# scychon/openmm_drudeNose

Hardware: AMD Instinct MI355X
Metric: integrator steps/sec at 1M Drude pairs (higher is better)
Workload: dtype f64; 1 GPU; SWM4-NDP water box, 1000000 molecules = 5000000 particle slots, 1000000 Drude pairs, 1 temperature group (+ molecular-COM and Drude thermostats), TGNH mode, mixed precision, numNHChains=1, hard wall 0.02 nm, harness force call-out inside the timed region (harness_force: lattice); harness_force=lattice, precision=mixed, variant=resident, hipgraph=False, parallelism=particle-sharded x1 (whole molecules), one KE all-reduce per step, slots_per_gpu=5000000

## Files before the change

### include/drude_tgnh.h

```cpp
#ifndef DRUDE_TGNH_H_
#define DRUDE_TGNH_H_

#include <stdint.h>

#ifdef __cplusplus
extern "C" {
#endif

#define TGNH_ABI_VERSION 1

typedef int tgnh_status;
enum {
    TGNH_OK = 0,
    TGNH_ERR_ARG = -1,
    TGNH_ERR_GROUP_MISMATCH = -2,
    TGNH_ERR_HARDWALL = -3,
    TGNH_ERR_UNSUPPORTED = -4,
    TGNH_ERR_HIP = -5,
    TGNH_ERR_STATE = -6
};

enum { TGNH_MODE_DUALNH = 0,
       TGNH_MODE_TGNH = 1 };

enum { TGNH_PREC_SINGLE = 0,
       TGNH_PREC_MIXED = 1,
       TGNH_PREC_DOUBLE = 2 };

enum { TGNH_FLAG_DEFER_SCALE = 2 };
enum { TGNH_FLAG_WAVE_TILES = 8 };
enum { TGNH_FLAG_RESIDENT_STEP = 4 };

enum { TGNH_FLAG_TRUST_STATE_CHANGED = 16 };

enum { TGNH_FLAG_GATHER = 32 };

typedef struct tgnh_desc {
    uint32_t struct_size;
    int32_t mode;
    int32_t precision;
    int32_t flags;
    int32_t device;
    int32_t num_particles;
    int32_t padded_num_particles;
    int32_t num_pairs;
    int32_t num_groups;
    int32_t num_residues;
    int32_t num_constraints;
    int32_t has_cm_motion_remover;
    const double* mass;
    const int32_t* pair_drude;
    const int32_t* pair_parent;
    const int32_t* group;
    const int32_t* resid;
    const int32_t* constraint_i;
    const int32_t* constraint_j;
    double kB;
    double temperature, coupling_time;
    double drude_temperature, drude_coupling_time;
    double step_size;
    int32_t drude_steps_per_real_step;
    int32_t num_nh_chains;
    int32_t use_drude_nh_chains;
    int32_t use_com_temp_group;
    double max_drude_distance;
} tgnh_desc;

typedef struct tgnh_context* tgnh_handle;


typedef int (*tgnh_allreduce_fn)(void* buf, int count, void* stream, void* user);

const char* tgnh_last_error(void);
int tgnh_abi_version(void);

tgnh_status tgnh_create(const tgnh_desc* desc, tgnh_handle* out);
tgnh_status tgnh_destroy(tgnh_handle h);

tgnh_status tgnh_bind_buffers(tgnh_handle h, void* posq, void* posq_correction, void* velm,
                              const void* force, void* pos_delta);

tgnh_status tgnh_set_step_size(tgnh_handle h, double dt);
tgnh_status tgnh_set_drude_steps_per_real_step(tgnh_handle h, int n);
tgnh_status tgnh_set_max_drude_distance(tgnh_handle h, double d);

tgnh_status tgnh_get_local_dof_terms(tgnh_handle h, double* terms, int* count);
tgnh_status tgnh_set_global_dof_terms(tgnh_handle h, const double* terms, int count);
tgnh_status tgnh_set_allreduce(tgnh_handle h, tgnh_allreduce_fn fn, void* user);

#define TGNH_RCCL_ID_BYTES 128
tgnh_status tgnh_rccl_unique_id(void* id_out);
tgnh_status tgnh_rccl_init(tgnh_handle h, int world, int rank, const void* id);
tgnh_status tgnh_set_rccl_comm(tgnh_handle h, void* nccl_comm);
tgnh_status tgnh_rccl_shutdown(tgnh_handle h);
tgnh_status tgnh_set_resident_share(tgnh_handle h, int share);
tgnh_status tgnh_get_resident_work_groups(tgnh_handle h, int* per_compute_unit);
tgnh_status tgnh_get_step_path(tgnh_handle h, int* gather, const char** reason);
tgnh_status tgnh_get_resident_kernel(tgnh_handle h, int* which);

#define TGNH_XCHG_HANDLE_BYTES 64
tgnh_status tgnh_exchange_create(tgnh_handle h, int world, int rank, void* ipc_handle_out, void** mailbox_out);
tgnh_status tgnh_exchange_attach(tgnh_handle h, const void* ipc_handles);
tgnh_status tgnh_exchange_attach_pointers(tgnh_handle h, void* const* mailboxes);
tgnh_status tgnh_exchange_detach(tgnh_handle h);
tgnh_status tgnh_exchange_wait_stats(tgnh_handle h, void* stream, double* mean_us, double* max_us, int64_t* exchanges);

tgnh_status tgnh_step_begin(tgnh_handle h, void* stream);
tgnh_status tgnh_step_end(tgnh_handle h, void* stream);
tgnh_status tgnh_step_begin_kick(tgnh_handle h, void* stream);
tgnh_status tgnh_step_begin_move(tgnh_handle h, void* stream);
tgnh_status tgnh_step_end_kick(tgnh_handle h, void* stream);
tgnh_status tgnh_step_end_thermo(tgnh_handle h, void* stream);
tgnh_status tgnh_flush(tgnh_handle h, void* stream);
tgnh_status tgnh_note_replayed_steps(tgnh_handle h, int nsteps);
tgnh_status tgnh_get_pending_state(tgnh_handle h, uint32_t* bits);
tgnh_status tgnh_set_time(tgnh_handle h, double time, int64_t step_count);
tgnh_status tgnh_state_changed(tgnh_handle h);

tgnh_status tgnh_get_kinetic_energy(tgnh_handle h, int ke_sum_valid, void* stream, double* out);
tgnh_status tgnh_get_num_thermostats(tgnh_handle h, int* count);
tgnh_status tgnh_get_last_kinetic_energies(tgnh_handle h, void* stream, double* ke);
tgnh_status tgnh_get_last_scale_factors(tgnh_handle h, void* stream, double* scale);
tgnh_status tgnh_get_status_flags(tgnh_handle h, void* stream, uint32_t* flags);
tgnh_status tgnh_get_time(tgnh_handle h, double* time, int64_t* step_count);
tgnh_status tgnh_get_dof(tgnh_handle h, double* dof, double* nkt);

tgnh_status tgnh_get_thermostat_len(tgnh_handle h, int which, int* len);
tgnh_status tgnh_get_thermostat_state(tgnh_handle h, int which, void* stream, double* out);
tgnh_status tgnh_set_thermostat_state(tgnh_handle h, int which, void* stream, const double* in);

tgnh_status tgnh_get_topology_len(tgnh_handle h, int which, int* len);
tgnh_status tgnh_get_topology(tgnh_handle h, int which, int32_t* out);
tgnh_status tgnh_get_launch_bounds(tgnh_handle h, int32_t out[8]);

tgnh_status tgnh_compute_kinetic_energies(tgnh_handle h, void* stream);
tgnh_status tgnh_half_kick(tgnh_handle h, void* stream);

tgnh_status tgnh_harness_force(tgnh_handle h, const void* x0, double k_drude, double k_tether,
                               void* force_out, void* stream);
tgnh_status tgnh_harness_pack_sites(tgnh_handle h, const void* x0);
tgnh_status tgnh_harness_lattice_hint(tgnh_handle h, int mol_slots, int side, double spacing, const double* geom, int first_molecule);
tgnh_status tgnh_harness_sites_kind(tgnh_handle h, int* kind);
tgnh_status tgnh_run_steps(tgnh_handle h, int nsteps, void* stream);
tgnh_status tgnh_run_harness(tgnh_handle h, const void* x0, double k_drude, double k_tether,
                             int nsteps, void* stream);

tgnh_status tgnh_harness_set_clusters(tgnh_handle h, int n, const int32_t* atoms, const double* dist);
tgnh_status tgnh_harness_shake_positions(tgnh_handle h, double tol, void* stream);
tgnh_status tgnh_harness_shake_velocities(tgnh_handle h, double tol, void* stream);
tgnh_status tgnh_harness_set_virtual_sites(tgnh_handle h, int n, const int32_t* atoms, const double* weights);
tgnh_status tgnh_harness_virtual_sites(tgnh_handle h, void* stream);
tgnh_status tgnh_run_harness_constrained(tgnh_handle h, const void* x0, double k_drude, double k_tether,
                                         double tol, int nsteps, void* stream);

tgnh_status tgnh_harness_water_force(tgnh_handle h, double box, double cutoff, void* force_out, void* stream);
tgnh_status tgnh_harness_remove_cm_motion(tgnh_handle h, void* stream);

tgnh_status tgnh_timing_enable(tgnh_handle h, int on);
tgnh_status tgnh_timing_read(tgnh_handle h, int kernel, double* total_ms, int64_t* launches);
tgnh_status tgnh_algorithmic_bytes(tgnh_handle h, int kernel, double* bytes);

#ifdef __cplusplus
}
#endif
#endif
```

### openmm_drudenose_amd/_lib.py

```python
import ctypes as C
import os

HERE = os.path.dirname(os.path.abspath(__file__))
LIB_PATH = os.environ.get("TGNH_LIB") or os.path.join(HERE, "libdrudetgnh_hip.so")

TGNH_OK = 0
ERR_ARG, ERR_GROUP_MISMATCH, ERR_HARDWALL, ERR_UNSUPPORTED, ERR_HIP, ERR_STATE = -1, -2, -3, -4, -5, -6
MODE_DUALNH, MODE_TGNH = 0, 1
PREC_SINGLE, PREC_MIXED, PREC_DOUBLE = 0, 1, 2
FLAG_DEFER_SCALE, FLAG_RESIDENT_STEP, FLAG_WAVE_TILES, FLAG_TRUST_STATE_CHANGED, FLAG_GATHER = 2, 4, 8, 16, 32
KID_SKD, KID_KICK_KE, KID_SCALE, KID_KE, KID_CHAIN, KID_FORCE, KID_OTHER, KID_STEP = range(8)
KERNEL_NAMES = {KID_SKD: "scale+kick+drift", KID_KICK_KE: "kick+KE", KID_SCALE: "rescale", KID_KE: "KE",
                KID_CHAIN: "chain", KID_FORCE: "harness force", KID_OTHER: "other", KID_STEP: "resident step"}

c_i32p = C.POINTER(C.c_int32)
c_f64p = C.POINTER(C.c_double)


class TgnhDesc(C.Structure):
    _fields_ = [
        ("struct_size", C.c_uint32), ("mode", C.c_int32), ("precision", C.c_int32), ("flags", C.c_int32),
        ("device", C.c_int32), ("num_particles", C.c_int32), ("padded_num_particles", C.c_int32),
        ("num_pairs", C.c_int32), ("num_groups", C.c_int32), ("num_residues", C.c_int32),
        ("num_constraints", C.c_int32), ("has_cm_motion_remover", C.c_int32),
        ("mass", c_f64p), ("pair_drude", c_i32p), ("pair_parent", c_i32p), ("group", c_i32p), ("resid", c_i32p),
        ("constraint_i", c_i32p), ("constraint_j", c_i32p),
        ("kB", C.c_double), ("temperature", C.c_double), ("coupling_time", C.c_double),
        ("drude_temperature", C.c_double), ("drude_coupling_time", C.c_double), ("step_size", C.c_double),
        ("drude_steps_per_real_step", C.c_int32), ("num_nh_chains", C.c_int32),
        ("use_drude_nh_chains", C.c_int32), ("use_com_temp_group", C.c_int32),
        ("max_drude_distance", C.c_double),
    ]


ALLREDUCE_FN = C.CFUNCTYPE(C.c_int, C.c_void_p, C.c_int, C.c_void_p, C.c_void_p)

SIGNATURES = {
    "tgnh_last_error": (C.c_char_p, []),
    "tgnh_abi_version": (C.c_int, []),
    "tgnh_create": (C.c_int, [C.POINTER(TgnhDesc), C.POINTER(C.c_void_p)]),
    "tgnh_destroy": (C.c_int, [C.c_void_p]),
    "tgnh_bind_buffers": (C.c_int, [C.c_void_p] * 6),
    "tgnh_set_step_size": (C.c_int, [C.c_void_p, C.c_double]),
    "tgnh_set_drude_steps_per_real_step": (C.c_int, [C.c_void_p, C.c_int]),
    "tgnh_set_max_drude_distance": (C.c_int, [C.c_void_p, C.c_double]),
    "tgnh_get_local_dof_terms": (C.c_int, [C.c_void_p, c_f64p, C.POINTER(C.c_int)]),
    "tgnh_set_global_dof_terms": (C.c_int, [C.c_void_p, c_f64p, C.c_int]),
    "tgnh_set_allreduce": (C.c_int, [C.c_void_p, ALLREDUCE_FN, C.c_void_p]),
    "tgnh_rccl_unique_id": (C.c_int, [C.c_void_p]),
    "tgnh_rccl_init": (C.c_int, [C.c_void_p, C.c_int, C.c_int, C.c_void_p]),
    "tgnh_set_rccl_comm": (C.c_int, [C.c_void_p, C.c_void_p]),
    "tgnh_rccl_shutdown": (C.c_int, [C.c_void_p]),
    "tgnh_exchange_wait_stats": (C.c_int, [C.c_void_p, C.c_void_p, c_f64p, c_f64p, C.POINTER(C.c_int64)]),
    "tgnh_get_pending_state": (C.c_int, [C.c_void_p, C.POINTER(C.c_uint32)]),
    "tgnh_set_resident_share": (C.c_int, [C.c_void_p, C.c_int]),
    "tgnh_get_resident_work_groups": (C.c_int, [C.c_void_p, C.POINTER(C.c_int)]),
    "tgnh_get_resident_kernel": (C.c_int, [C.c_void_p, C.POINTER(C.c_int)]),
    "tgnh_get_step_path": (C.c_int, [C.c_void_p, C.POINTER(C.c_int), C.POINTER(C.c_char_p)]),
    "tgnh_exchange_create": (C.c_int, [C.c_void_p, C.c_int, C.c_int, C.c_void_p, C.POINTER(C.c_void_p)]),
    "tgnh_exchange_attach": (C.c_int, [C.c_void_p, C.c_char_p]),
    "tgnh_exchange_attach_pointers": (C.c_int, [C.c_void_p, C.POINTER(C.c_void_p)]),
    "tgnh_exchange_detach": (C.c_int, [C.c_void_p]),
    "tgnh_step_begin": (C.c_int, [C.c_void_p, C.c_void_p]),
    "tgnh_step_end": (C.c_int, [C.c_void_p, C.c_void_p]),
    "tgnh_step_begin_kick": (C.c_int, [C.c_void_p, C.c_void_p]),
    "tgnh_step_begin_move": (C.c_int, [C.c_void_p, C.c_void_p]),
    "tgnh_step_end_kick": (C.c_int, [C.c_void_p, C.c_void_p]),
    "tgnh_step_end_thermo": (C.c_int, [C.c_void_p, C.c_void_p]),
    "tgnh_flush": (C.c_int, [C.c_void_p, C.c_void_p]),
    "tgnh_state_changed": (C.c_int, [C.c_void_p]),
    "tgnh_note_replayed_steps": (C.c_int, [C.c_void_p, C.c_int]),
    "tgnh_set_time": (C.c_int, [C.c_void_p, C.c_double, C.c_int64]),
    "tgnh_get_kinetic_energy": (C.c_int, [C.c_void_p, C.c_int, C.c_void_p, c_f64p]),
    "tgnh_get_num_thermostats": (C.c_int, [C.c_void_p, C.POINTER(C.c_int)]),
    "tgnh_get_last_kinetic_energies": (C.c_int, [C.c_void_p, C.c_void_p, c_f64p]),
    "tgnh_get_last_scale_factors": (C.c_int, [C.c_void_p, C.c_void_p, c_f64p]),
    "tgnh_get_status_flags": (C.c_int, [C.c_void_p, C.c_void_p, C.POINTER(C.c_uint32)]),
    "tgnh_get_time": (C.c_int, [C.c_void_p, c_f64p, C.POINTER(C.c_int64)]),
    "tgnh_get_dof": (C.c_int, [C.c_void_p, c_f64p, c_f64p]),
    "tgnh_get_thermostat_len": (C.c_int, [C.c_void_p, C.c_int, C.POINTER(C.c_int)]),
    "tgnh_get_thermostat_state": (C.c_int, [C.c_void_p, C.c_int, C.c_void_p, c_f64p]),
    "tgnh_set_thermostat_state": (C.c_int, [C.c_void_p, C.c_int, C.c_void_p, c_f64p]),
    "tgnh_get_topology_len": (C.c_int, [C.c_void_p, C.c_int, C.POINTER(C.c_int)]),
    "tgnh_get_topology": (C.c_int, [C.c_void_p, C.c_int, c_i32p]),
    "tgnh_get_launch_bounds": (C.c_int, [C.c_void_p, c_i32p]),
    "tgnh_compute_kinetic_energies": (C.c_int, [C.c_void_p, C.c_void_p]),
    "tgnh_half_kick": (C.c_int, [C.c_void_p, C.c_void_p]),
    "tgnh_harness_force": (C.c_int, [C.c_void_p, C.c_void_p, C.c_double, C.c_double, C.c_void_p, C.c_void_p]),
    "tgnh_harness_pack_sites": (C.c_int, [C.c_void_p, C.c_void_p]),
    "tgnh_harness_lattice_hint": (C.c_int, [C.c_void_p, C.c_int, C.c_int, C.c_double, c_f64p, C.c_int]),
    "tgnh_harness_sites_kind": (C.c_int, [C.c_void_p, C.POINTER(C.c_int)]),
    "tgnh_run_harness": (C.c_int, [C.c_void_p, C.c_void_p, C.c_double, C.c_double, C.c_int, C.c_void_p]),
    "tgnh_run_steps": (C.c_int, [C.c_void_p, C.c_int, C.c_void_p]),
    "tgnh_harness_set_clusters": (C.c_int, [C.c_void_p, C.c_int, c_i32p, c_f64p]),
    "tgnh_harness_shake_positions": (C.c_int, [C.c_void_p, C.c_double, C.c_void_p]),
    "tgnh_harness_shake_velocities": (C.c_int, [C.c_void_p, C.c_double, C.c_void_p]),
    "tgnh_harness_set_virtual_sites": (C.c_int, [C.c_void_p, C.c_int, c_i32p, c_f64p]),
    "tgnh_harness_virtual_sites": (C.c_int, [C.c_void_p, C.c_void_p]),
    "tgnh_run_harness_constrained": (C.c_int, [C.c_void_p, C.c_void_p, C.c_double, C.c_double, C.c_double, C.c_int, C.c_void_p]),
    "tgnh_harness_water_force": (C.c_int, [C.c_void_p, C.c_double, C.c_double, C.c_void_p, C.c_void_p]),
    "tgnh_harness_remove_cm_motion": (C.c_int, [C.c_void_p, C.c_void_p]),
    "tgnh_timing_enable": (C.c_int, [C.c_void_p, C.c_int]),
    "tgnh_timing_read": (C.c_int, [C.c_void_p, C.c_int, c_f64p, C.POINTER(C.c_int64)]),
    "tgnh_algorithmic_bytes": (C.c_int, [C.c_void_p, C.c_int, c_f64p]),
}

_lib = None


def load():
    global _lib
    if _lib is not None:
        return _lib
    if not os.path.exists(LIB_PATH):
        raise RuntimeError(
            f"{LIB_PATH} is missing: build it with `python -m openmm_drudenose_amd.build` "
            "(hipcc --offload-arch=gfx950). There is no CPU fallback for the integrator path.")
    try:
        import torch
    except ImportError:
        pass
    lib = C.CDLL(LIB_PATH)
    for name, (res, args) in SIGNATURES.items():
        if os.environ.get("TGNH_LIB") and not hasattr(lib, name):
            continue
        fn = getattr(lib, name)
        fn.restype = res
        fn.argtypes = args
    _lib = lib
    return lib
```

### openmm_drudenose_amd/csrc/tgnh_context.h

```cpp
#ifndef TGNH_CONTEXT_H_
#define TGNH_CONTEXT_H_

#include <map>
#include <string>
#include <vector>

#include "tgnh_internal.h"

void tgnh_set_error(const std::string& msg);

namespace tgnh {
template <typename T> class DeviceBuf {
    T* p_ = nullptr;
    bool pinned_ = false;
public:
    DeviceBuf() = default;
    DeviceBuf(DeviceBuf&& o) noexcept : p_(o.p_), pinned_(o.pinned_) { o.p_ = nullptr; }
    ~DeviceBuf() { reset(); }
    void reset() { if (p_) (void)(pinned_ ? hipHostFree(p_) : hipFree(p_)); p_ = nullptr; }
    hipError_t alloc(size_t n, bool zero = false, unsigned ext_flags = 0) {
        reset(); pinned_ = false;
        void* p = nullptr;
        hipError_t e = ext_flags ? hipExtMallocWithFlags(&p, sizeof(T) * n, ext_flags) : hipMalloc(&p, sizeof(T) * n);
        if (e != hipSuccess) return e;
        p_ = static_cast<T*>(p);
        return zero ? hipMemset(p_, 0, sizeof(T) * n) : hipSuccess;
    }
    hipError_t alloc_pinned(size_t n) { reset(); pinned_ = true; return hipHostMalloc(reinterpret_cast<void**>(&p_), sizeof(T) * n, hipHostMallocDefault); }
    hipError_t upload(const T* src, size_t n) {
        hipError_t e = alloc(n ? n : 1);
        return e != hipSuccess || !n ? e : hipMemcpy(p_, src, sizeof(T) * n, hipMemcpyHostToDevice);
    }
    hipError_t upload(const std::vector<T>& v) { return upload(v.data(), v.size()); }
    T* get() const { return p_; }
    operator T*() const { return p_; }
};
typedef DeviceBuf<unsigned char> DeviceBytes;
}

struct tgnh_context {
    tgnh_desc d;
    int device = 0;
    bool host_only = false;
    struct Topology {
        std::vector<double> mass;
        std::vector<int> pair_drude, pair_parent, group, resid, normal;
        std::vector<int> res_count, res_first;
        std::vector<int> tile_start, tile_res;
        std::vector<int2> res_entries;
        std::vector<int> big_first, big_count;
        int num_big = 0, num_tiles = 0;
        std::vector<uint32_t> meta;
        std::vector<int2> wave_tile;
        std::vector<uint32_t> wmeta;
        std::vector<uint32_t> tile_pat, wtile_pat;
        std::vector<uint32_t> pattern, wpattern;
        int num_wtiles = 0;
        tgnh::DeviceBuf<uint32_t> d_meta, d_wmeta, d_tile_pat, d_pattern, d_wpattern;
        tgnh::DeviceBuf<int> d_tile_start, d_tile_res;
        tgnh::DeviceBuf<int2> d_res_table, d_wave_tile, d_big_table;
        tgnh::DeviceBytes d_big_com;
    } topo;
    struct Gather {
        bool generic = false;
        bool chain = false;
        std::string reason;
        std::vector<int2> res_table;
        std::vector<int> resid, partner;
        int com_lanes = 64;
        tgnh::DeviceBuf<int> d_group, d_resid, d_partner;
        tgnh::DeviceBuf<int2> d_res_table;
        tgnh::DeviceBytes d_com;
        tgnh::DeviceBuf<double> d_scratch;
    } gather;
    struct Thermostat {
        std::vector<double> h_state;
        std::vector<double> local_terms, global_terms;
        std::vector<double> dof, nkbt;
        double realkbT = 0, drudekbT = 0;
        tgnh::ChainLayout L{};
        tgnh::DeviceBuf<double> d_partials;
        tgnh::DeviceBuf<double> d_state;
        tgnh::DeviceBuf<double> d_stage;
        tgnh::DeviceBuf<double> d_scalar;
    } thermo;
    struct LaunchConfig {
        int grid = 0, gb = 1;
        int num_cus = 256, grid_override = 0;
        std::map<int, int> grid_cache;
        bool alternate_sweeps = true;
        int inline_sum_rows = tgnh::CHAIN_INLINE_SUM_ROWS;
        bool inline_sum_all = false;
        bool carry_ok = false;
        bool inline_chain = false;
        bool wave_ke = false;
        int resident_grid[5][2] = {{0, 0}, {0, 0}, {0, 0}, {0, 0}, {0, 0}};
        int resident_share = 1;
        int wresident_per_cu = 0, wresident_grid = 0;
        int resident_per_cu = 0;
    } cfg;
    struct Owed {
        bool end_pending = false;
        bool scale_pending = false;
        bool kick_pending = false;
        bool first_half_done = false;
        bool chain_pending = false;
        bool sum_pending = false;
        bool xwait_pending = false;
        bool stage_pending = false;
        bool ke_carry = false;
        bool chain_pending_twice = false;
        bool carry_pending = false;
        bool tail_summed = false;
        bool end_folded = false;
        bool g_com_fresh = false;
        enum : uint32_t { BIT_SWEEP_REVERSE = 1u << 8 };
        uint32_t bits() const {
            return end_pending | scale_pending << 1 | kick_pending << 2 | first_half_done << 3 | chain_pending << 4 | sum_pending << 5 |
                   xwait_pending << 6 | stage_pending << 7 | ke_carry << 9;
        }
        void chain_owed(bool twice) { chain_pending = true; chain_pending_twice = twice; }
        void chain_ran() { chain_pending = sum_pending = xwait_pending = carry_pending = false; }
        void velocities_current() { scale_pending = kick_pending = false; }
        void end_half_deferred(bool kick) { scale_pending = first_half_done = true; kick_pending = kick; }
        void resident_settled() { end_pending = first_half_done = false; velocities_current(); chain_pending = sum_pending = xwait_pending = false; }
        void thermostat_reset() { end_pending = first_half_done = false; velocities_current(); chain_pending = stage_pending = carry_pending = ke_carry = false; }
    } owed;
    struct Run {
        double time = 0;
        int64_t step_count = 0;
        int sweep_reverse = 0;
        int ke_parts = 0;
    } run;
    struct Bound {
        void *posq = nullptr, *posq_corr = nullptr, *velm = nullptr, *pos_delta = nullptr;
        const void* force = nullptr;
    } bound;
    struct Status {
        tgnh::DeviceBuf<uint32_t> d_word;
        tgnh::DeviceBuf<uint32_t> h_seen;
        int failed_code = 0;
        std::string failed;
    } status;
    struct Meeting {
        tgnh::DeviceBuf<unsigned int> d_sync;
        tgnh::DeviceBuf<unsigned long long> d_rows;
        tgnh::DeviceBuf<unsigned long long> self_box;
        tgnh::DeviceBuf<unsigned long long> d_self_misc;
        tgnh::XchgArgs self_x{};
    } meet;
    struct Exchange {
        tgnh_allreduce_fn allreduce = nullptr;
        void* allreduce_user = nullptr;
        void* rccl_comm = nullptr;
        bool rccl_owned = false;
        tgnh::XchgArgs args{};
        bool on = false;
        int world = 0, rank = 0;
        tgnh::DeviceBuf<unsigned long long> mailbox;
        tgnh::DeviceBuf<unsigned long long*> d_peers;
        std::vector<void*> opened;
        tgnh::DeviceBuf<unsigned long long> d_seq;
        tgnh::DeviceBuf<unsigned int> d_dead;
        tgnh::DeviceBuf<unsigned long long> d_stat;
        void close_peers() { for (void* p : opened) (void)hipIpcCloseMemHandle(p); opened.clear(); }
        ~Exchange() { close_peers(); }
    } xchg;
    struct Harness {
        tgnh::DeviceBuf<int4> d_cl_atoms, d_vs_atoms;
        tgnh::DeviceBuf<double> d_cl_dist, d_vs_w;
        int num_clusters = 0, num_sites = 0;
        tgnh::DeviceBuf<uint8_t> d_sflag;
        tgnh::DeviceBuf<uint32_t> d_sbase;
        tgnh::DeviceBytes d_sites;
        int lat_k = 0, lat_side = 0, lat_mol0 = 0;
        double lat_spacing = 0;
        std::vector<double> lat_geom;
        bool lat_on = false;
        tgnh::DeviceBuf<unsigned char> d_lat_tab;
        tgnh::DeviceBytes d_g_x0;
    } harness;
    struct Timing {
        bool on = false;
        int only = -1;
        struct Ev { hipEvent_t a, b; int kid; };
        std::vector<Ev> ev_pool;
        size_t ev_used = 0;
        double t_total[tgnh::KID_COUNT] = {0};
        int64_t t_count[tgnh::KID_COUNT] = {0};
        ~Timing() { for (auto& e : ev_pool) { (void)hipEventDestroy(e.a); (void)hipEventDestroy(e.b); } }
    } timing;
};

#endif
```

### openmm_drudenose_amd/csrc/tgnh_exchange.cpp

```cpp
#include <dlfcn.h>
#include <mutex>
#if __has_include(<rccl/rccl.h>)
#include <rccl/rccl.h>
#else
extern "C" {
typedef struct ncclComm* ncclComm_t;
typedef struct { char internal[128]; } ncclUniqueId;
typedef enum { ncclSuccess = 0 } ncclResult_t;
typedef enum { ncclSum = 0 } ncclRedOp_t;
typedef enum { ncclDouble = 8 } ncclDataType_t;
}
#endif

#include "tgnh_host.h"

extern "C" tgnh_status tgnh_exchange_create(tgnh_handle h, int world, int rank, void* ipc_handle_out, void** mailbox_out) {
    CHECK_H(h);
    if (h->host_only) return fail(TGNH_ERR_STATE, "host-only handle");
    if (world < 1 || world > XCHG_MAX_WORLD || rank < 0 || rank >= world) return fail(TGNH_ERR_ARG, "bad world / rank");
    if (h->thermo.L.NT > MAX_GROUPS + 2) return fail(TGNH_ERR_UNSUPPORTED, "too many thermostats for a mailbox (more than 32 temperature groups: use an all-reduce hook or RCCL)");
    if (h->gather.chain) return fail(TGNH_ERR_UNSUPPORTED, "no mailbox for a chain too long for the LDS-resident form (it runs in gather_chain_kernel: use an all-reduce hook or RCCL)");
    if (h->xchg.mailbox) return fail(TGNH_ERR_STATE, "exchange already created");
    HIP_OK(hipSetDevice(h->device));
    HIP_OK(h->xchg.mailbox.alloc(XCHG_MAILBOX_BYTES(world) / sizeof(unsigned long long), true, hipDeviceMallocUncached));
    HIP_OK(h->xchg.d_seq.alloc(1, true));
    HIP_OK(h->xchg.d_dead.alloc(1, true));
    HIP_OK(h->xchg.d_peers.alloc(world));
    HIP_OK(h->xchg.d_stat.alloc(3, true));
    HIP_OK(hipDeviceSynchronize());
    h->xchg.world = world; h->xchg.rank = rank;
    if (ipc_handle_out) {
        static_assert(sizeof(hipIpcMemHandle_t) == TGNH_XCHG_HANDLE_BYTES, "IPC handle size");
        hipIpcMemHandle_t ih;
        HIP_OK(hipIpcGetMemHandle(&ih, h->xchg.mailbox));
        std::memcpy(ipc_handle_out, &ih, sizeof(ih));
    }
    if (mailbox_out) *mailbox_out = h->xchg.mailbox;
    return TGNH_OK;
}

static tgnh_status exchange_finish_attach(tgnh_handle h, const std::vector<unsigned long long*>& peers) {
    HIP_OK(hipMemcpy(h->xchg.d_peers, peers.data(), sizeof(unsigned long long*) * peers.size(), hipMemcpyHostToDevice));
    h->xchg.args = XchgArgs{};
    h->xchg.args.on = 1; h->xchg.args.world = h->xchg.world; h->xchg.args.rank = h->xchg.rank;
    h->xchg.args.peers = h->xchg.d_peers; h->xchg.args.mine = h->xchg.mailbox; h->xchg.args.seq = h->xchg.d_seq; h->xchg.args.dead = h->xchg.d_dead;
    h->xchg.args.status = h->status.d_word;
    h->xchg.args.stat = h->xchg.d_stat;
    h->xchg.on = true;
    return TGNH_OK;
}

extern "C" tgnh_status tgnh_exchange_attach(tgnh_handle h, const void* ipc_handles) {
    CHECK_H(h);
    if (!h->xchg.mailbox) return fail(TGNH_ERR_STATE, "tgnh_exchange_create first");
    if (!ipc_handles) return fail(TGNH_ERR_ARG, "null handles");
    tgnh_status rc = deferred_guard(h, "tgnh_exchange_attach"); if (rc) return rc;
    h->owed.ke_carry = false;
    HIP_OK(hipSetDevice(h->device));
    std::vector<unsigned long long*> peers(h->xchg.world, nullptr);
    for (int r = 0; r < h->xchg.world; r++) {
        if (r == h->xchg.rank) { peers[r] = h->xchg.mailbox; continue; }
        hipIpcMemHandle_t ih;
        std::memcpy(&ih, static_cast<const char*>(ipc_handles) + (size_t)r * TGNH_XCHG_HANDLE_BYTES, sizeof(ih));
        void* p = nullptr;
        HIP_OK(hipIpcOpenMemHandle(&p, ih, hipIpcMemLazyEnablePeerAccess));
        h->xchg.opened.push_back(p);
        peers[r] = static_cast<unsigned long long*>(p);
    }
    return exchange_finish_attach(h, peers);
}

extern "C" tgnh_status tgnh_exchange_attach_pointers(tgnh_handle h, void* const* mailboxes) {
    CHECK_H(h);
    if (!h->xchg.mailbox) return fail(TGNH_ERR_STATE, "tgnh_exchange_create first");
    if (!mailboxes) return fail(TGNH_ERR_ARG, "null mailboxes");
    tgnh_status rc = deferred_guard(h, "tgnh_exchange_attach_pointers"); if (rc) return rc;
    h->owed.ke_carry = false;
    HIP_OK(hipSetDevice(h->device));
    std::vector<unsigned long long*> peers(h->xchg.world, nullptr);
    for (int r = 0; r < h->xchg.world; r++) {
        peers[r] = r == h->xchg.rank ? h->xchg.mailbox : static_cast<unsigned long long*>(mailboxes[r]);
        if (!peers[r]) return fail(TGNH_ERR_ARG, "null mailbox pointer");
    }
    return exchange_finish_attach(h, peers);
}

extern "C" tgnh_status tgnh_exchange_detach(tgnh_handle h) {
    CHECK_H(h);
    if (!h->xchg.on) return TGNH_OK;
    HIP_OK(hipSetDevice(h->device));
    HIP_OK(hipDeviceSynchronize());
    {
        uint32_t f = 0;
        HIP_OK(hipMemcpy(&f, h->status.d_word, sizeof(uint32_t), hipMemcpyDeviceToHost));
        note_status(h, f);
    }
    if (h->owed.end_pending && !h->status.failed_code) {
        tgnh_status rc = settle_end(h, (hipStream_t)0); if (rc) return rc;
        HIP_OK(hipDeviceSynchronize());
    }
    if (h->owed.chain_pending && h->owed.xwait_pending && !h->status.failed_code) {
        tgnh_status rc = materialize_chain(h, (hipStream_t)0); if (rc) return rc;
        HIP_OK(hipDeviceSynchronize());
    }
    h->xchg.on = false;
    h->xchg.close_peers();
    return TGNH_OK;
}

extern "C" tgnh_status tgnh_set_allreduce(tgnh_handle h, tgnh_allreduce_fn fn, void* user) {
    CHECK_H(h);
    tgnh_status rc = deferred_guard(h, "tgnh_set_allreduce"); if (rc) return rc;
    h->owed.ke_carry = false;
    if (h->xchg.rccl_comm) { rc = tgnh_rccl_shutdown(h); if (rc) return rc; }
    h->xchg.allreduce = fn; h->xchg.allreduce_user = user;
    return TGNH_OK;
}

namespace {
struct Rccl {
    void* lib = nullptr;
    ncclResult_t (*GetUniqueId)(ncclUniqueId*) = nullptr;
    ncclResult_t (*CommInitRank)(ncclComm_t*, int, ncclUniqueId, int) = nullptr;
    ncclResult_t (*CommDestroy)(ncclComm_t) = nullptr;
    ncclResult_t (*AllReduce)(const void*, void*, size_t, ncclDataType_t, ncclRedOp_t, ncclComm_t, hipStream_t) = nullptr;
    const char* (*GetErrorString)(ncclResult_t) = nullptr;
    std::string error;
    bool ok = false;
};
void rccl_bind(Rccl& r);
Rccl& rccl() {
    static Rccl r;
    static std::once_flag once;
    std::call_once(once, [] { rccl_bind(r); });
    return r;
}
void rccl_bind(Rccl& r) {
    const char* names[] = {"librccl.so.1", "librccl.so", "/opt/rocm/lib/librccl.so.1"};
    for (const char* n : names) if (!r.lib) r.lib = dlopen(n, RTLD_NOW | RTLD_NOLOAD);
    for (const char* n : names) if (!r.lib) r.lib = dlopen(n, RTLD_NOW | RTLD_LOCAL);
    if (!r.lib) { r.error = std::string("RCCL not found (librccl.so.1): ") + dlerror(); return; }
    r.GetUniqueId = reinterpret_cast<decltype(r.GetUniqueId)>(dlsym(r.lib, "ncclGetUniqueId"));
    r.CommInitRank = reinterpret_cast<decltype(r.CommInitRank)>(dlsym(r.lib, "ncclCommInitRank"));
    r.CommDestroy = reinterpret_cast<decltype(r.CommDestroy)>(dlsym(r.lib, "ncclCommDestroy"));
    r.AllReduce = reinterpret_cast<decltype(r.AllReduce)>(dlsym(r.lib, "ncclAllReduce"));
    r.GetErrorString = reinterpret_cast<decltype(r.GetErrorString)>(dlsym(r.lib, "ncclGetErrorString"));
    r.ok = r.GetUniqueId && r.CommInitRank && r.CommDestroy && r.AllReduce && r.GetErrorString;
    if (!r.ok) r.error = "RCCL: a required symbol is missing from librccl";
}
#define RCCL_OK(expr)                                                                                        \
    do {                                                                                                     \
        ncclResult_t r_ = (expr);                                                                            \
        if (r_ != ncclSuccess) return fail(TGNH_ERR_HIP, std::string(#expr) + ": " + rccl().GetErrorString(r_)); \
    } while (0)

int rccl_allreduce(void* buf, int count, void* stream, void* user) {
    tgnh_context* h = static_cast<tgnh_context*>(user);
    return rccl().AllReduce(buf, buf, (size_t)count, ncclDouble, ncclSum, static_cast<ncclComm_t>(h->xchg.rccl_comm),
                            static_cast<hipStream_t>(stream)) == ncclSuccess ? 0 : 1;
}
}

extern "C" tgnh_status tgnh_rccl_unique_id(void* id_out) {
    if (!id_out) return fail(TGNH_ERR_ARG, "null id");
    static_assert(sizeof(ncclUniqueId) == TGNH_RCCL_ID_BYTES, "ncclUniqueId size");
    if (!rccl().ok) return fail(TGNH_ERR_HIP, rccl().error);
    ncclUniqueId id;
    RCCL_OK(rccl().GetUniqueId(&id));
    std::memcpy(id_out, &id, sizeof(id));
    return TGNH_OK;
}

extern "C" tgnh_status tgnh_set_rccl_comm(tgnh_handle h, void* nccl_comm) {
    CHECK_H(h);
    if (h->host_only) return fail(TGNH_ERR_STATE, "host-only handle");
    tgnh_status rc = deferred_guard(h, "tgnh_set_rccl_comm"); if (rc) return rc;
    h->owed.ke_carry = false;
    if (!rccl().ok) return fail(TGNH_ERR_HIP, rccl().error);
    if (h->xchg.rccl_comm) { rc = tgnh_rccl_shutdown(h); if (rc) return rc; }
    if (!nccl_comm) {
        if (h->xchg.allreduce == rccl_allreduce) { h->xchg.allreduce = nullptr; h->xchg.allreduce_user = nullptr; }
        return TGNH_OK;
    }
    h->xchg.rccl_comm = nccl_comm; h->xchg.rccl_owned = false;
    h->xchg.allreduce = rccl_allreduce; h->xchg.allreduce_user = h;
    return TGNH_OK;
}

extern "C" tgnh_status tgnh_rccl_init(tgnh_handle h, int world, int rank, const void* id) {
    CHECK_H(h);
    if (h->host_only) return fail(TGNH_ERR_STATE, "host-only handle");
    if (world < 1 || rank < 0 || rank >= world || !id) return fail(TGNH_ERR_ARG, "bad world / rank / id");
    tgnh_status rc = deferred_guard(h, "tgnh_rccl_init"); if (rc) return rc;
    h->owed.ke_carry = false;
    if (!rccl().ok) return fail(TGNH_ERR_HIP, rccl().error);
    if (h->xchg.rccl_comm) { rc = tgnh_rccl_shutdown(h); if (rc) return rc; }
    HIP_OK(hipSetDevice(h->device));
    ncclUniqueId uid;
    std::memcpy(&uid, id, sizeof(uid));
    ncclComm_t comm = nullptr;
    RCCL_OK(rccl().CommInitRank(&comm, world, uid, rank));
    h->xchg.rccl_comm = comm; h->xchg.rccl_owned = true;
    h->xchg.allreduce = rccl_allreduce; h->xchg.allreduce_user = h;
    return TGNH_OK;
}

extern "C" tgnh_status tgnh_rccl_shutdown(tgnh_handle h) {
    CHECK_H(h);
    if (!h->xchg.rccl_comm) return TGNH_OK;
    if (!h->host_only) { HIP_OK(hipSetDevice(h->device)); HIP_OK(hipDeviceSynchronize()); }
    if (h->xchg.allreduce == rccl_allreduce) { h->xchg.allreduce = nullptr; h->xchg.allreduce_user = nullptr; }
    ncclComm_t comm = static_cast<ncclComm_t>(h->xchg.rccl_comm);
    const bool owned = h->xchg.rccl_owned;
    h->xchg.rccl_comm = nullptr; h->xchg.rccl_owned = false;
    if (owned) RCCL_OK(rccl().CommDestroy(comm));
    return TGNH_OK;
}

extern "C" tgnh_status tgnh_get_resident_work_groups(tgnh_handle h, int* per_compute_unit) {
    CHECK_H(h);
    if (!per_compute_unit) return fail(TGNH_ERR_ARG, "null out");
    *per_compute_unit = resident_now(h) ? std::max(h->cfg.resident_per_cu, h->cfg.wresident_per_cu) : 0;
    return TGNH_OK;
}

extern "C" tgnh_status tgnh_exchange_wait_stats(tgnh_handle h, void* stream, double* mean_us, double* max_us, int64_t* exchanges) {
    CHECK_H(h);
    if (!h->xchg.d_stat) return fail(TGNH_ERR_STATE, "tgnh_exchange_create first");
    HIP_OK(hipSetDevice(h->device));
    unsigned long long st[3] = {0, 0, 0};
    hipStream_t s = (hipStream_t)stream;
    HIP_OK(hipMemcpyAsync(st, h->xchg.d_stat, sizeof(st), hipMemcpyDeviceToHost, s));
    HIP_OK(hipMemsetAsync(h->xchg.d_stat, 0, sizeof(st), s));
    HIP_OK(hipStreamSynchronize(s));
    const double tick_us = 0.01;
    if (mean_us) *mean_us = st[2] ? tick_us * (double)st[0] / (double)st[2] : 0.0;
    if (max_us) *max_us = tick_us * (double)st[1];
    if (exchanges) *exchanges = (int64_t)st[2];
    return TGNH_OK;
}

extern "C" tgnh_status tgnh_set_resident_share(tgnh_handle h, int share) {
    CHECK_H(h);
    if (share < 1 || share > 64) return fail(TGNH_ERR_ARG, "resident share must be 1..64");
    h->cfg.resident_share = share;
    h->cfg.wresident_grid = 0;
    for (auto& g : h->cfg.resident_grid) g[0] = g[1] = 0;
    return TGNH_OK;
}
```

### openmm_drudenose_amd/csrc/tgnh_harness_host.cpp

```cpp
#include "tgnh_host.h"

extern "C" tgnh_status tgnh_harness_force(tgnh_handle h, const void* x0, double k_drude, double k_tether,
                                          void* force_out, void* stream) {
    tgnh_status rc = entry(h, true); if (rc) return rc;
    if (!force_out) return fail(TGNH_ERR_ARG, "null force_out");
    if (h->gather.generic) {
        if (!x0) x0 = h->harness.d_g_x0;
        if (!x0) return fail(TGNH_ERR_ARG, "null x0 and no packed sites (tgnh_harness_pack_sites)");
        Timed t(h, (hipStream_t)stream, KID_FORCE);
        HIP_OK(launch_gather_force(h->d.precision, gather_args(h, nullptr), x0, reinterpret_cast<long long*>(force_out), k_drude, k_tether, (hipStream_t)stream));
        return TGNH_OK;
    }
    if (!x0 && !h->harness.d_sflag && !h->harness.lat_on) return fail(TGNH_ERR_ARG, "null x0 and no packed sites (tgnh_harness_pack_sites)");
    ForceArgs a{};
    a.posq = h->bound.posq; a.posq_corr = h->bound.posq_corr; a.x0 = x0; a.meta = h->topo.d_meta;
    if (!x0 && h->harness.lat_on) {
        a.lat_k = h->harness.lat_k; a.lat_side = h->harness.lat_side; a.lat_mol0 = h->harness.lat_mol0; a.lat_spacing = h->harness.lat_spacing; a.lat_tab = h->harness.d_lat_tab;
        a.lat_inv_k = 1.0 / h->harness.lat_k; a.lat_inv_side = 1.0 / h->harness.lat_side; a.lat_inv_side2 = 1.0 / ((double)h->harness.lat_side * h->harness.lat_side);
    } else if (!x0) { a.sflag = h->harness.d_sflag; a.sbase = h->harness.d_sbase; a.sites = h->harness.d_sites; }
    a.force = reinterpret_cast<long long*>(force_out);
    a.n = h->d.num_particles; a.padded = h->d.padded_num_particles;
    a.k_drude = k_drude; a.k_tether = k_tether;
    a.reverse = h->run.sweep_reverse;
    if (h->cfg.alternate_sweeps) h->run.sweep_reverse ^= 1;
    Timed t(h, (hipStream_t)stream, KID_FORCE);
    HIP_OK(launch_force(h->d.precision, a, (hipStream_t)stream));
    return TGNH_OK;
}

extern "C" tgnh_status tgnh_harness_pack_sites(tgnh_handle h, const void* x0) {
    tgnh_status rc = entry(h, false); if (rc) return rc;
    if (h->host_only) return fail(TGNH_ERR_STATE, "host-only handle");
    if (!x0) return fail(TGNH_ERR_ARG, "null x0");
    const int N = h->d.num_particles;
    const size_t rs = h->d.precision == TGNH_PREC_DOUBLE ? sizeof(double) : sizeof(float);
    if (h->gather.generic) {
        h->harness.lat_on = false;
        if (!h->harness.d_g_x0) HIP_OK(h->harness.d_g_x0.alloc((size_t)std::max(N, 1) * 4 * rs));
        HIP_OK(hipMemcpy(h->harness.d_g_x0, x0, (size_t)N * 4 * rs, hipMemcpyDeviceToDevice));
        return TGNH_OK;
    }
    std::vector<unsigned char> raw((size_t)std::max(N, 1) * 4 * rs);
    HIP_OK(hipMemcpy(raw.data(), x0, (size_t)N * 4 * rs, hipMemcpyDeviceToHost));
    std::vector<uint8_t> flag((size_t)std::max(N, 1), 0);
    std::vector<uint32_t> base((size_t)(N + 63) / 64 + 1, 0);
    std::vector<unsigned char> sites;
    sites.reserve((size_t)N * 3 * rs);
    uint32_t count = 0;
    for (int i = 0; i < N; i++) {
        if ((i & 63) == 0) base[i >> 6] = count;
        const unsigned char* rec = raw.data() + (size_t)i * 4 * rs;
        const bool tethered = rs == sizeof(double) ? reinterpret_cast<const double*>(rec)[3] != 0.0 : reinterpret_cast<const float*>(rec)[3] != 0.0f;
        const uint32_t m = h->topo.meta[i], role = m & 3u;
        const int off = (int)((m >> 10) & 2047u) - 1024;
        const uint32_t o5 = role == ROLE_NORMAL ? 16u : (off >= -15 && off <= 15 ? (uint32_t)(off + 16) : 0u);
        flag[i] = (uint8_t)(role | (tethered && role != ROLE_DRUDE ? 4u : 0u) | (o5 << 3));
        if (flag[i] & 4u) { sites.insert(sites.end(), rec, rec + 3 * rs); count++; }
    }
    h->harness.d_sflag.reset(); h->harness.d_sbase.reset(); h->harness.d_sites.reset();
    h->harness.lat_on = false;
    if (h->harness.lat_k > 0) {
        const int k = h->harness.lat_k, side = h->harness.lat_side;
        bool ok = N > 0 && N % k == 0 && (long long)side * side * side >= (long long)h->harness.lat_mol0 + N / k;
        for (int i = 0; i < N && ok; i++) {
            const int pos = i % k, mol = h->harness.lat_mol0 + i / k;
            ok = flag[i] == flag[pos] && (flag[i] >> 3) != 0;
            if (ok && (flag[i] & 4u)) {
                const int idx[3] = {mol / (side * side), (mol / side) % side, mol % side};
                const unsigned char* rec = raw.data() + (size_t)i * 4 * rs;
                for (int ax = 0; ax < 3 && ok; ax++) {
                    volatile double c = (double)idx[ax] * h->harness.lat_spacing;
                    const double v = c + h->harness.lat_geom[(size_t)pos * 3 + ax];
                    ok = rs == sizeof(double) ? reinterpret_cast<const double*>(rec)[ax] == v : reinterpret_cast<const float*>(rec)[ax] == (float)v;
                }
            }
        }
        if (ok) {
            std::vector<unsigned char> tab(LAT_TAB_BYTES, 0);
            std::memcpy(tab.data(), flag.data(), (size_t)k);
            std::memcpy(tab.data() + 64, h->harness.lat_geom.data(), sizeof(double) * 3 * (size_t)k);
            HIP_OK(h->harness.d_lat_tab.upload(tab));
            h->harness.lat_on = true;
            return TGNH_OK;
        }
    }
    HIP_OK(h->harness.d_sflag.upload(flag));
    HIP_OK(h->harness.d_sbase.upload(base));
    HIP_OK(h->harness.d_sites.alloc(std::max(sites.size(), (size_t)16) + 16));
    if (!sites.empty()) HIP_OK(hipMemcpy(h->harness.d_sites, sites.data(), sites.size(), hipMemcpyHostToDevice));
    return TGNH_OK;
}

extern "C" tgnh_status tgnh_harness_lattice_hint(tgnh_handle h, int mol_slots, int side, double spacing, const double* geom, int first_molecule) {
    CHECK_H(h);
    h->harness.lat_on = false;
    if (mol_slots == 0) { h->harness.lat_k = 0; h->harness.lat_geom.clear(); return TGNH_OK; }
    if (mol_slots < 1 || mol_slots > 64 || side < 1 || side > 1290 || !(spacing > 0) || !geom || first_molecule < 0) return fail(TGNH_ERR_ARG, "bad lattice hint");
    h->harness.lat_k = mol_slots; h->harness.lat_side = side; h->harness.lat_spacing = spacing; h->harness.lat_mol0 = first_molecule;
    h->harness.lat_geom.assign(geom, geom + 3 * (size_t)mol_slots);
    return TGNH_OK;
}
extern "C" tgnh_status tgnh_harness_sites_kind(tgnh_handle h, int* kind) {
    CHECK_H(h);
    if (!kind) return fail(TGNH_ERR_ARG, "null out");
    *kind = h->harness.lat_on ? 2 : (h->harness.d_sflag ? 1 : 0);
    return TGNH_OK;
}

extern "C" tgnh_status tgnh_run_harness(tgnh_handle h, const void* x0, double k_drude, double k_tether,
                                        int nsteps, void* stream) {
    CHECK_H(h);
    for (int i = 0; i < nsteps; i++) {
        tgnh_status rc = tgnh_step_begin(h, stream); if (rc) return rc;
        rc = tgnh_harness_force(h, x0, k_drude, k_tether, const_cast<void*>(h->bound.force), stream); if (rc) return rc;
        rc = tgnh_step_end(h, stream); if (rc) return rc;
    }
    return TGNH_OK;
}

extern "C" tgnh_status tgnh_run_steps(tgnh_handle h, int nsteps, void* stream) {
    CHECK_H(h);
    for (int i = 0; i < nsteps; i++) {
        tgnh_status rc = tgnh_step_begin(h, stream); if (rc) return rc;
        rc = tgnh_step_end(h, stream); if (rc) return rc;
    }
    return TGNH_OK;
}
```

### openmm_drudenose_amd/csrc/tgnh_host.h

```cpp
#ifndef TGNH_HOST_H_
#define TGNH_HOST_H_

#include <algorithm>
#include <cmath>
#include <cstdio>
#include <cstdlib>
#include <cstring>

#include "tgnh_context.h"

using namespace tgnh;

#pragma GCC visibility push(hidden)
inline tgnh_status fail(tgnh_status code, const std::string& msg) {
    tgnh_set_error(msg);
    return code;
}
#define HIP_OK(expr) do { hipError_t e_ = (expr); if (e_ != hipSuccess) return fail(TGNH_ERR_HIP, std::string(#expr) + ": " + hipGetErrorString(e_)); } while (0)
#define CHECK_H(h) do { if (!(h)) return fail(TGNH_ERR_ARG, "null handle"); } while (0)

inline bool com_thermostat_on(const tgnh_desc& d) { return d.mode == TGNH_MODE_TGNH && d.use_com_temp_group; }
inline int pass_kind(const tgnh_desc& d) { return (d.flags & TGNH_FLAG_DEFER_SCALE) ? 0 : 1; }
void make_layout(tgnh_context* c);
tgnh_status build_topology(tgnh_context* c, const tgnh_desc* d);
void local_dof_terms(tgnh_context* c);
tgnh_status finalize_thermostat(tgnh_context* c);
tgnh_status deferred_guard(tgnh_handle h, const char* what);
void note_status(tgnh_handle h, uint32_t flags);
tgnh_status entry(tgnh_handle h, bool need_bufs);
bool resident_now(tgnh_handle h);
tgnh_status allreduce_hook(tgnh_handle h, hipStream_t s);
tgnh_status run_tile(tgnh_handle h, int ops, int kid, hipStream_t s, const double* scale = nullptr);
GatherArgs gather_args(tgnh_handle h, const double* scale);
ChainArgs chain_args(tgnh_handle h);
tgnh_status run_chain_gather(tgnh_handle h, hipStream_t s, bool sum_only);
tgnh_status materialize_chain(tgnh_handle h, hipStream_t s);
tgnh_status settle_kick(tgnh_handle h, hipStream_t s);
tgnh_status settle_end(tgnh_handle h, hipStream_t s);
tgnh_status flush_impl(tgnh_handle h, hipStream_t s);

struct Timed {
    tgnh_context* c; hipStream_t s; int kid; tgnh_context::Timing::Ev* ev = nullptr;
    Timed(tgnh_context* c_, hipStream_t s_, int kid_) : c(c_), s(s_), kid(kid_) {
        if (!c->timing.on) return;
        if (c->timing.only >= 0 && kid != c->timing.only) return;
        if (c->timing.ev_used == c->timing.ev_pool.size()) {
            tgnh_context::Timing::Ev e; e.kid = kid;
            if (hipEventCreate(&e.a) != hipSuccess || hipEventCreate(&e.b) != hipSuccess) return;
            c->timing.ev_pool.push_back(e);
        }
        ev = &c->timing.ev_pool[c->timing.ev_used++];
        ev->kid = kid;
        (void)hipEventRecord(ev->a, s);
    }
    ~Timed() { if (ev) (void)hipEventRecord(ev->b, s); }
};
#pragma GCC visibility pop

#endif
```

### openmm_drudenose_amd/csrc/tgnh_lifecycle.cpp

```cpp
#include <memory>

#include "tgnh_host.h"
#ifndef TGNH_MEETING_MEM
#define TGNH_MEETING_MEM hipDeviceMallocFinegrained
#endif

static thread_local std::string g_err;
extern "C" const char* tgnh_last_error(void) { return g_err.c_str(); }
extern "C" int tgnh_abi_version(void) { return TGNH_ABI_VERSION; }

void tgnh_set_error(const std::string& msg) { g_err = msg; }

static tgnh_status validate_desc(const tgnh_desc* d, bool* long_chain) {
    if (d->struct_size != sizeof(tgnh_desc)) return fail(TGNH_ERR_ARG, "tgnh_desc size mismatch (ABI)");
    if (d->mode != TGNH_MODE_DUALNH && d->mode != TGNH_MODE_TGNH) return fail(TGNH_ERR_ARG, "bad mode");
    if (d->precision < TGNH_PREC_SINGLE || d->precision > TGNH_PREC_DOUBLE) return fail(TGNH_ERR_ARG, "bad precision");
    if (d->num_particles < 1 || d->num_pairs < 0 || !d->mass || (d->num_pairs && (!d->pair_drude || !d->pair_parent)))
        return fail(TGNH_ERR_ARG, "bad particle / pair arrays");
    if (d->padded_num_particles < d->num_particles) return fail(TGNH_ERR_ARG, "padded_num_particles < num_particles");
    if (d->num_constraints < 0) return fail(TGNH_ERR_ARG, "negative num_constraints");
    if (3LL * d->padded_num_particles > 2147483647LL)
        return fail(TGNH_ERR_UNSUPPORTED, "more than 715 827 882 padded particle slots: the index into the third force plane leaves 32 bits");
    if (d->num_nh_chains < 1 || d->drude_steps_per_real_step < 1) return fail(TGNH_ERR_ARG, "numNHChains and drudeStepsPerRealStep must be >= 1");
    if (d->mode == TGNH_MODE_TGNH && (d->num_groups < 1 || d->num_residues < 1 || !d->group || !d->resid))
        return fail(TGNH_ERR_ARG, "TGNH mode needs temperature groups and residues");
    if (!(d->max_drude_distance >= 0)) return fail(TGNH_ERR_ARG, "setMaxDrudeDistance: Distance cannot be negative");
    if (d->flags & ~(uint32_t)(TGNH_FLAG_DEFER_SCALE | TGNH_FLAG_RESIDENT_STEP | TGNH_FLAG_WAVE_TILES | TGNH_FLAG_TRUST_STATE_CHANGED | TGNH_FLAG_GATHER))
        return fail(TGNH_ERR_ARG, "unknown bits in tgnh_desc.flags (a newer header than this library?)");
    if (d->mode == TGNH_MODE_DUALNH && d->num_pairs == 0)
        return fail(TGNH_ERR_UNSUPPORTED, "dualNH mode needs at least one Drude pair (the Reference platform does too)");
    if (!(d->step_size > 0) || !std::isfinite(d->step_size)) return fail(TGNH_ERR_ARG, "step size must be positive");
    *long_chain = false;
    {
        const long need = d->mode == TGNH_MODE_TGNH ? (long)(d->num_groups + 2) * (4L * d->num_nh_chains + 1)
                                                    : 4L * (2L * d->num_nh_chains + 4);
        if (d->num_nh_chains > (d->mode == TGNH_MODE_TGNH ? 16 : 4) && need > 2048) {
            if (d->mode != TGNH_MODE_TGNH) return fail(TGNH_ERR_UNSUPPORTED, "numNHChains too large for the on-device chain");
            *long_chain = true;
        }
    }
    return TGNH_OK;
}

static tgnh_status decide_policy(tgnh_context* c, const tgnh_desc* d, bool long_chain) {
    if (c->gather.generic) {
        c->d.flags &= ~(TGNH_FLAG_DEFER_SCALE | TGNH_FLAG_RESIDENT_STEP | TGNH_FLAG_TRUST_STATE_CHANGED | TGNH_FLAG_WAVE_TILES);
        c->gather.chain = c->d.mode == TGNH_MODE_TGNH && (c->thermo.L.NT > MAX_GROUPS + 2 || long_chain);
    }
    c->cfg.wave_ke = !c->gather.generic && !c->topo.wave_tile.empty() && c->cfg.gb != 0 &&
                 ((d->flags & TGNH_FLAG_WAVE_TILES) || (double)d->num_particles >= 0.9 * WAVE_SLOTS * (double)c->topo.num_wtiles);
#ifdef TGNH_TUNING
    if (const char* e = getenv("TGNH_WAVE_KE")) c->cfg.wave_ke = c->cfg.wave_ke && e[0] != '0';
#endif
    {
        bool inside = true;
        if (com_thermostat_on(*d)) {
            std::vector<int> g0(d->num_residues, -1);
            for (int i = 0; i < d->num_particles && inside; i++) {
                if (c->topo.mass[i] == 0.0) continue;
                int& g = g0[c->topo.resid[i]];
                if (g == -1) g = c->topo.group[i];
                else if (g != c->topo.group[i]) inside = false;
            }
        }
        if ((c->d.flags & TGNH_FLAG_DEFER_SCALE) && !inside) return fail(TGNH_ERR_UNSUPPORTED, "DEFER_SCALE needs every molecule inside one temperature group");
        c->cfg.carry_ok = (c->d.flags & TGNH_FLAG_TRUST_STATE_CHANGED) && !(c->d.flags & TGNH_FLAG_DEFER_SCALE) && inside;
    }
    c->cfg.grid = GRID_CAP;
#ifdef TGNH_TUNING
    if (const char* e = getenv("TGNH_GRID")) { int g = atoi(e); if (g >= 1) c->cfg.grid_override = std::min(g, GRID_CAP); }
#endif
    {
        bool want = true;
        c->cfg.inline_sum_all = d->num_particles < 2000000;
#ifdef TGNH_TUNING
        if (const char* e = getenv("TGNH_INLINE_CHAIN")) want = e[0] != '0';
        if (const char* e4 = getenv("TGNH_INLINE_SUM_ROWS")) c->cfg.inline_sum_rows = atoi(e4);
        if (const char* e5 = getenv("TGNH_INLINE_SUM_ALL")) c->cfg.inline_sum_all = e5[0] != '0';
        if (const char* e3 = getenv("TGNH_ALTERNATE_SWEEPS")) c->cfg.alternate_sweeps = e3[0] != '0';
#endif
        int inline_multi_max = 2500000;
#ifdef TGNH_TUNING
        if (const char* e6 = getenv("TGNH_INLINE_MULTI_MAX")) inline_multi_max = atoi(e6);
#endif
        c->cfg.inline_chain = want && !c->gather.generic && (c->thermo.L.C == 1 || (c->thermo.L.C <= 4 && d->num_particles < inline_multi_max));
        if (c->thermo.L.total > 256 && c->thermo.L.C > 1) c->cfg.inline_chain = c->cfg.inline_chain && false;
    }
    return TGNH_OK;
}

static tgnh_status allocate(tgnh_context* c) {
    const size_t NT = c->thermo.L.NT;
    HIP_OK(c->thermo.d_partials.alloc((size_t)(c->cfg.grid + c->topo.num_big) * NT, true));
    HIP_OK(c->thermo.d_state.alloc(c->thermo.L.total));
    HIP_OK(c->thermo.d_stage.alloc(c->thermo.L.total));
    HIP_OK(c->status.d_word.alloc(1, true));
    HIP_OK(c->status.h_seen.alloc_pinned(1));
    *c->status.h_seen = 0;
    if (c->gather.chain && c->thermo.L.C > 4) HIP_OK(c->gather.d_scratch.alloc(NT * (4 * c->thermo.L.C + 1)));
    HIP_OK(c->thermo.d_scalar.alloc(1 + PLAIN_KE_PARTS));
    HIP_OK(c->meet.d_sync.alloc(4, true));
    const bool resident = (c->d.flags & TGNH_FLAG_RESIDENT_STEP) != 0;
    if (c->cfg.wave_ke || resident)
        HIP_OK(c->meet.d_rows.alloc(2 * (size_t)GRID_CAP * CHAIN_INLINE_SUM_NT, true, TGNH_MEETING_MEM));
    if (!resident) return TGNH_OK;
    HIP_OK(c->meet.self_box.alloc(XCHG_MAILBOX_BYTES(1) / sizeof(unsigned long long), true, TGNH_MEETING_MEM));
    HIP_OK(c->meet.d_self_misc.alloc(4, true));
    unsigned long long* const box = c->meet.self_box;
    HIP_OK(hipMemcpy(c->meet.d_self_misc + 2, &box, sizeof(box), hipMemcpyHostToDevice));
    c->meet.self_x = XchgArgs{};
    c->meet.self_x.on = 1; c->meet.self_x.world = 1; c->meet.self_x.rank = 0;
    c->meet.self_x.peers = reinterpret_cast<unsigned long long* const*>(c->meet.d_self_misc + 2);
    c->meet.self_x.mine = c->meet.self_box;
    c->meet.self_x.seq = c->meet.d_self_misc;
    c->meet.self_x.dead = reinterpret_cast<unsigned int*>(c->meet.d_self_misc + 1);
    c->meet.self_x.status = c->status.d_word;
    return TGNH_OK;
}

template <typename Launch> static tgnh_status census(tgnh_context* c, int per_cu_max, Launch&& launch, int* found) {
    for (int per_cu = std::min(per_cu_max, 8); per_cu >= 1 && !*found; per_cu--) {
        TileArgs a{};
        a.census = 1; a.sync = c->meet.d_sync;
        HIP_OK(hipMemset(c->meet.d_sync + 2, 0, 2 * sizeof(unsigned int)));
        const int grid = std::min(per_cu * c->cfg.num_cus, GRID_CAP);
        HIP_OK(launch(a, grid));
        unsigned int res[2] = {0, 1};
        HIP_OK(hipMemcpy(res, c->meet.d_sync + 2, sizeof(res), hipMemcpyDeviceToHost));
        if (res[0] == (unsigned)grid && res[1] == 0) *found = per_cu;
    }
    return TGNH_OK;
}

static tgnh_status resident_census(tgnh_context* c) {
    if (!(c->d.flags & TGNH_FLAG_RESIDENT_STEP) || c->cfg.gb == 0 || !c->cfg.inline_chain || c->thermo.L.NT > CHAIN_INLINE_SUM_NT) return TGNH_OK;
    const int kind = pass_kind(c->d);
    const size_t lds = tile_lds_bytes(c->d.precision, step_kind_ops2(kind), true, true);
    tgnh_status rc = census(c, c->thermo.L.C == 1 ? step_blocks_per_cu(c->d.precision, c->cfg.gb, kind, lds) : 0,
                            [&](const TileArgs& a, int grid) { return launch_step(c->d.precision, c->cfg.gb, kind, a, grid, lds, (hipStream_t)0); },
                            &c->cfg.resident_per_cu);
    if (rc) return rc;
    const bool multi = c->thermo.L.C > 1;
    bool want_w = c->cfg.wave_ke && (c->d.flags & TGNH_FLAG_DEFER_SCALE) && (c->cfg.resident_per_cu > 0 || multi);
    if (c->d.mode == TGNH_MODE_DUALNH && !c->thermo.L.use_drude_chains && multi) want_w = false;
#ifdef TGNH_TUNING
    if (const char* e = getenv("TGNH_WSTEP")) want_w = want_w && e[0] != '0';
#endif
    return census(c, want_w ? wstep_blocks_per_cu(c->d.precision, c->cfg.gb, multi) : 0,
                  [&](const TileArgs& a, int grid) { return launch_wstep(c->d.precision, c->cfg.gb, multi, a, grid, (hipStream_t)0); },
                  &c->cfg.wresident_per_cu);
}

extern "C" tgnh_status tgnh_create(const tgnh_desc* d, tgnh_handle* out) {
    if (!d || !out) return fail(TGNH_ERR_ARG, "null argument");
    bool long_chain = false;
    tgnh_status rc = validate_desc(d, &long_chain); if (rc) return rc;
    const bool host_only = d->device == -1;
    if (!host_only) {
        int ndev = 0;
        HIP_OK(hipGetDeviceCount(&ndev));
        if (d->device < 0 || d->device >= ndev) return fail(TGNH_ERR_HIP, "no such HIP device (the HIP path needs an MI355X; there is no CPU fallback)");
        HIP_OK(hipSetDevice(d->device));
    }

    std::unique_ptr<tgnh_context> owner(new tgnh_context());
    tgnh_context* c = owner.get();
    c->host_only = host_only;
    c->d = *d;
    c->device = d->device;
    c->thermo.realkbT = d->kB * d->temperature;
    c->thermo.drudekbT = d->kB * d->drude_temperature;
    make_layout(c);
    c->cfg.gb = c->thermo.L.G <= 1 ? 1 : (c->thermo.L.G <= 4 ? 4 : (c->thermo.L.G <= 8 ? 8 : 0));
    if (long_chain) { c->gather.generic = true; c->gather.reason = "a chain too long for the LDS-resident form"; }
    else if (d->flags & TGNH_FLAG_GATHER) { c->gather.generic = true; c->gather.reason = "asked for (TGNH_FLAG_GATHER)"; }
    if (!host_only) {
        hipDeviceProp_t prop;
        if (hipGetDeviceProperties(&prop, d->device) == hipSuccess && prop.multiProcessorCount > 0) c->cfg.num_cus = prop.multiProcessorCount;
    }
    rc = build_topology(c, d); if (rc) return rc;
    rc = decide_policy(c, d, long_chain); if (rc) return rc;
    local_dof_terms(c);
    c->thermo.global_terms = c->thermo.local_terms;
    c->d.mass = nullptr; c->d.pair_drude = c->d.pair_parent = c->d.group = c->d.resid = nullptr;
    c->d.constraint_i = c->d.constraint_j = nullptr;

    if (!host_only) {
        rc = allocate(c); if (rc) return rc;
        rc = resident_census(c); if (rc) return rc;
    }
    rc = finalize_thermostat(c); if (rc) return rc;
    *out = owner.release();
    return TGNH_OK;
}

extern "C" tgnh_status tgnh_destroy(tgnh_handle h) {
    CHECK_H(h);
    if (h->xchg.rccl_comm) (void)tgnh_rccl_shutdown(h);
    if (!h->host_only) (void)hipSetDevice(h->device);
    delete h;
    return TGNH_OK;
}

extern "C" tgnh_status tgnh_bind_buffers(tgnh_handle h, void* posq, void* posq_correction, void* velm,
                                         const void* force, void* pos_delta) {
    CHECK_H(h);
    if (h->host_only) return fail(TGNH_ERR_STATE, "host-only handle (device -1): no GPU work can be launched on it");
    if (!posq || !velm || !force) return fail(TGNH_ERR_ARG, "posq, velm and force are required");
    if (h->d.precision == TGNH_PREC_MIXED && !posq_correction) return fail(TGNH_ERR_ARG, "mixed precision needs posqCorrection");
    if ((h->owed.kick_pending || h->owed.end_pending) && (velm != h->bound.velm || force != h->bound.force))
        return fail(TGNH_ERR_STATE, "tgnh_bind_buffers: velm / force may not be rebound while a deferred half kick is pending (tgnh_flush first)");
    if (posq == h->bound.posq && posq_correction == h->bound.posq_corr && velm == h->bound.velm && force == h->bound.force && pos_delta == h->bound.pos_delta)
        return TGNH_OK;
    {
        HIP_OK(hipSetDevice(h->device));
        const size_t N = (size_t)h->d.num_particles, P = (size_t)h->d.padded_num_particles;
        const size_t r4 = h->d.precision == TGNH_PREC_DOUBLE ? 32 : 16, m4 = h->d.precision == TGNH_PREC_SINGLE ? 16 : 32;
        struct { const void* p; size_t need; const char* name; } bufs[] = {
            {posq, N * r4, "posq"}, {posq_correction, N * 16, "posqCorrection"}, {velm, N * m4, "velm"},
            {force, 3 * P * sizeof(long long), "force"}, {pos_delta, N * m4, "posDelta"}};
        for (const auto& b : bufs) {
            if (!b.p) continue;
            hipDeviceptr_t base = nullptr; size_t size = 0;
            if (hipMemGetAddressRange(&base, &size, const_cast<void*>(b.p)) != hipSuccess) { (void)hipGetLastError(); continue; }
            const size_t left = size - (size_t)(static_cast<const char*>(b.p) - static_cast<const char*>(base));
            if (left < b.need)
                return fail(TGNH_ERR_ARG, std::string("tgnh_bind_buffers: ") + b.name + " has " + std::to_string(left) + " bytes behind the pointer, the launches touch " + std::to_string(b.need));
        }
    }
    h->owed.ke_carry = false;
    h->bound.posq = posq; h->bound.posq_corr = posq_correction; h->bound.velm = velm; h->bound.force = force; h->bound.pos_delta = pos_delta;
    return TGNH_OK;
}

tgnh_status deferred_guard(tgnh_handle h, const char* what) {
    if (h->owed.first_half_done || h->owed.end_pending)
        return fail(TGNH_ERR_STATE, std::string(what) + ": not allowed between steps with TGNH_FLAG_DEFER_SCALE (the next thermostat half step has already run)");
    return TGNH_OK;
}

extern "C" tgnh_status tgnh_set_step_size(tgnh_handle h, double dt) {
    CHECK_H(h);
    if (!(dt > 0) || !std::isfinite(dt)) return fail(TGNH_ERR_ARG, "step size must be positive");
    if (dt != h->d.step_size) { tgnh_status rc = deferred_guard(h, "tgnh_set_step_size"); if (rc) return rc; }
    h->d.step_size = dt;
    return TGNH_OK;
}
extern "C" tgnh_status tgnh_set_drude_steps_per_real_step(tgnh_handle h, int n) {
    CHECK_H(h);
    if (n < 1) return fail(TGNH_ERR_ARG, "drudeStepsPerRealStep must be >= 1");
    if (n != h->d.drude_steps_per_real_step) { tgnh_status rc = deferred_guard(h, "tgnh_set_drude_steps_per_real_step"); if (rc) return rc; }
    h->d.drude_steps_per_real_step = n;
    return TGNH_OK;
}
extern "C" tgnh_status tgnh_set_max_drude_distance(tgnh_handle h, double dist) {
    CHECK_H(h);
    if (!(dist >= 0)) return fail(TGNH_ERR_ARG, "setMaxDrudeDistance: Distance cannot be negative");
    h->d.max_drude_distance = dist;
    return TGNH_OK;
}

extern "C" tgnh_status tgnh_get_local_dof_terms(tgnh_handle h, double* terms, int* count) {
    CHECK_H(h);
    if (count) *count = h->thermo.L.NT;
    if (terms) std::copy(h->thermo.local_terms.begin(), h->thermo.local_terms.end(), terms);
    return TGNH_OK;
}
extern "C" tgnh_status tgnh_set_global_dof_terms(tgnh_handle h, const double* terms, int count) {
    CHECK_H(h);
    if (!terms || count != h->thermo.L.NT) return fail(TGNH_ERR_ARG, "dof term count mismatch");
    if (h->run.step_count != 0) return fail(TGNH_ERR_STATE, "global dof must be set before the first step");
    if (!h->host_only) HIP_OK(hipSetDevice(h->device));
    h->thermo.global_terms.assign(terms, terms + count);
    return finalize_thermostat(h);
}
```

### openmm_drudenose_amd/csrc/tgnh_queries.cpp

```cpp
#include "tgnh_host.h"

static tgnh_status read_state(tgnh_handle h, int off, int n, hipStream_t s, double* out) {
    if (!out) return fail(TGNH_ERR_ARG, "null out");
    if (h->host_only) { std::copy(h->thermo.h_state.begin() + off, h->thermo.h_state.begin() + off + n, out); return TGNH_OK; }
    { tgnh_status rc = entry(h, false); if (rc) return rc; }
    { tgnh_status rc = materialize_chain(h, s); if (rc) return rc; }
    HIP_OK(hipMemcpyAsync(out, h->thermo.d_state + off, sizeof(double) * n, hipMemcpyDeviceToHost, s));
    HIP_OK(hipMemcpyAsync(h->status.h_seen, h->status.d_word, sizeof(uint32_t), hipMemcpyDeviceToHost, s));
    HIP_OK(hipStreamSynchronize(s));
    note_status(h, *h->status.h_seen);
    if (h->status.failed_code) return fail(h->status.failed_code, h->status.failed);
    return TGNH_OK;
}

extern "C" tgnh_status tgnh_get_kinetic_energy(tgnh_handle h, int ke_sum_valid, void* stream, double* out) {
    CHECK_H(h);
    if (!out) return fail(TGNH_ERR_ARG, "null out");
    hipStream_t s = (hipStream_t)stream;
    if (h->d.mode == TGNH_MODE_TGNH && ke_sum_valid)
        return read_state(h, h->thermo.L.off_kesum, 1, s, out);
    tgnh_status rc = entry(h, true); if (rc) return rc;
    rc = flush_impl(h, s); if (rc) return rc;
    const double ts = h->d.mode == TGNH_MODE_DUALNH ? 0.5 * h->d.step_size : 0.0;
    HIP_OK(launch_plain_ke(h->d.precision, h->bound.velm, reinterpret_cast<const long long*>(h->bound.force), h->d.num_particles,
                           h->d.padded_num_particles, ts, h->thermo.d_scalar, s));
    HIP_OK(hipMemcpyAsync(out, h->thermo.d_scalar, sizeof(double), hipMemcpyDeviceToHost, s));
    HIP_OK(hipStreamSynchronize(s));
    return TGNH_OK;
}

extern "C" tgnh_status tgnh_get_num_thermostats(tgnh_handle h, int* count) {
    CHECK_H(h);
    if (count) *count = h->thermo.L.NT;
    return TGNH_OK;
}
extern "C" tgnh_status tgnh_get_last_kinetic_energies(tgnh_handle h, void* stream, double* ke) {
    CHECK_H(h);
    return read_state(h, h->thermo.L.off_ke, h->thermo.L.NT, (hipStream_t)stream, ke);
}
extern "C" tgnh_status tgnh_get_last_scale_factors(tgnh_handle h, void* stream, double* scale) {
    CHECK_H(h);
    return read_state(h, h->thermo.L.off_scale_a, h->thermo.L.NT, (hipStream_t)stream, scale);
}
extern "C" tgnh_status tgnh_get_status_flags(tgnh_handle h, void* stream, uint32_t* flags) {
    CHECK_H(h);
    if (!flags) return fail(TGNH_ERR_ARG, "null flags");
    if (h->host_only) { *flags = 0; return TGNH_OK; }
    HIP_OK(hipSetDevice(h->device));
    HIP_OK(hipMemcpyAsync(h->status.h_seen, h->status.d_word, sizeof(uint32_t), hipMemcpyDeviceToHost, (hipStream_t)stream));
    HIP_OK(hipStreamSynchronize((hipStream_t)stream));
    *flags = *h->status.h_seen;
    note_status(h, *flags);
    if (h->status.failed_code) return fail(h->status.failed_code, h->status.failed);
    return TGNH_OK;
}
extern "C" tgnh_status tgnh_get_time(tgnh_handle h, double* time, int64_t* step_count) {
    CHECK_H(h);
    if (time) *time = h->run.time;
    if (step_count) *step_count = h->run.step_count;
    return TGNH_OK;
}
extern "C" tgnh_status tgnh_get_dof(tgnh_handle h, double* dof, double* nkt) {
    CHECK_H(h);
    if (dof) std::copy(h->thermo.dof.begin(), h->thermo.dof.end(), dof);
    if (nkt) std::copy(h->thermo.nkbt.begin(), h->thermo.nkbt.end(), nkt);
    return TGNH_OK;
}

static bool chain_section(tgnh_handle h, int which, int* off, int* len) {
    switch (which) {
        case 0: *off = h->thermo.L.off_eta; *len = h->thermo.L.len_eta; return true;
        case 1: *off = h->thermo.L.off_etaDot; *len = h->thermo.L.len_etaDot; return true;
        case 2: *off = h->thermo.L.off_etaDotDot; *len = h->thermo.L.len_etaDotDot; return true;
        case 3: *off = h->thermo.L.off_etaMass; *len = h->thermo.L.len_etaMass; return true;
        default: return false;
    }
}
extern "C" tgnh_status tgnh_get_thermostat_len(tgnh_handle h, int which, int* len) {
    CHECK_H(h);
    int off;
    if (!len) return fail(TGNH_ERR_ARG, "null out");
    if (!chain_section(h, which, &off, len)) return fail(TGNH_ERR_ARG, "bad thermostat array id");
    return TGNH_OK;
}
extern "C" tgnh_status tgnh_get_thermostat_state(tgnh_handle h, int which, void* stream, double* out) {
    CHECK_H(h);
    int off, len;
    if (!chain_section(h, which, &off, &len)) return fail(TGNH_ERR_ARG, "bad thermostat array id");
    return read_state(h, off, len, (hipStream_t)stream, out);
}
extern "C" tgnh_status tgnh_set_thermostat_state(tgnh_handle h, int which, void* stream, const double* in) {
    CHECK_H(h);
    int off, len;
    if (!chain_section(h, which, &off, &len)) return fail(TGNH_ERR_ARG, "bad thermostat array id");
    if (!in) return fail(TGNH_ERR_ARG, "null in");
    tgnh_status rc = deferred_guard(h, "tgnh_set_thermostat_state"); if (rc) return rc;
    h->owed.ke_carry = false;
    if (h->host_only) { std::copy(in, in + len, h->thermo.h_state.begin() + off); return TGNH_OK; }
    HIP_OK(hipSetDevice(h->device));
    rc = materialize_chain(h, (hipStream_t)stream); if (rc) return rc;
    HIP_OK(hipMemcpyAsync(h->thermo.d_state + off, in, sizeof(double) * len, hipMemcpyHostToDevice, (hipStream_t)stream));
    HIP_OK(hipMemcpyAsync(h->thermo.d_stage + off, in, sizeof(double) * len, hipMemcpyHostToDevice, (hipStream_t)stream));
    HIP_OK(hipStreamSynchronize((hipStream_t)stream));
    return TGNH_OK;
}

static const std::vector<int>* topo_vec(tgnh_handle h, int which) {
    switch (which) {
        case 0: return &h->topo.normal;
        case 1: return &h->topo.pair_drude;
        case 2: return &h->topo.pair_parent;
        case 3: return &h->topo.group;
        case 4: return &h->topo.resid;
        case 5: return &h->topo.res_count;
        case 6: return &h->topo.res_first;
        case 7: return &h->topo.tile_start;
        default: return nullptr;
    }
}
extern "C" tgnh_status tgnh_get_topology_len(tgnh_handle h, int which, int* len) {
    CHECK_H(h);
    if (!len) return fail(TGNH_ERR_ARG, "null out");
    if (which == 8) { *len = (int)h->topo.meta.size(); return TGNH_OK; }
    if (which == 9) { *len = 2 * (int)h->topo.wave_tile.size(); return TGNH_OK; }
    if (which == 10) { *len = (int)h->topo.wmeta.size(); return TGNH_OK; }
    if (which == 11) { *len = (int)h->topo.tile_pat.size(); return TGNH_OK; }
    if (which == 12) { *len = (int)h->topo.wtile_pat.size(); return TGNH_OK; }
    if (which == 13) { *len = (int)h->topo.pattern.size(); return TGNH_OK; }
    if (which == 14) { *len = (int)h->topo.wpattern.size(); return TGNH_OK; }
    const std::vector<int>* v = topo_vec(h, which);
    if (!v) return fail(TGNH_ERR_ARG, "bad topology array id");
    *len = (int)v->size();
    return TGNH_OK;
}
extern "C" tgnh_status tgnh_get_topology(tgnh_handle h, int which, int32_t* out) {
    CHECK_H(h);
    if (!out) return fail(TGNH_ERR_ARG, "null out");
    auto put = [&](const void* src, size_t bytes) { if (bytes) std::memcpy(out, src, bytes); return TGNH_OK; };
    if (which == 8) return put(h->topo.meta.data(), sizeof(uint32_t) * h->topo.meta.size());
    if (which == 9) return put(h->topo.wave_tile.data(), sizeof(int2) * h->topo.wave_tile.size());
    if (which == 10) return put(h->topo.wmeta.data(), sizeof(uint32_t) * h->topo.wmeta.size());
    if (which == 11) return put(h->topo.tile_pat.data(), sizeof(uint32_t) * h->topo.tile_pat.size());
    if (which == 12) return put(h->topo.wtile_pat.data(), sizeof(uint32_t) * h->topo.wtile_pat.size());
    if (which == 13) return put(h->topo.pattern.data(), sizeof(uint32_t) * h->topo.pattern.size());
    if (which == 14) return put(h->topo.wpattern.data(), sizeof(uint32_t) * h->topo.wpattern.size());
    const std::vector<int>* v = topo_vec(h, which);
    if (!v) return fail(TGNH_ERR_ARG, "bad topology array id");
    std::copy(v->begin(), v->end(), out);
    return TGNH_OK;
}

extern "C" tgnh_status tgnh_compute_kinetic_energies(tgnh_handle h, void* stream) {
    tgnh_status rc = entry(h, true); if (rc) return rc;
    hipStream_t s = (hipStream_t)stream;
    rc = settle_kick(h, s); if (rc) return rc;
    rc = materialize_chain(h, s); if (rc) return rc;
    const int dir = h->run.sweep_reverse;
    rc = run_tile(h, OP_KE, KID_KE, s);
    h->run.sweep_reverse = dir;
    if (rc) return rc;
    if (h->gather.chain) {
        rc = run_chain_gather(h, s, true); if (rc) return rc;
    } else {
        ChainArgs a = chain_args(h);
        a.do_sum = 1; a.do_chain = 0;
        if (h->xchg.on) { a.x_send = 1; a.x_wait = 1; }
        if (!h->owed.tail_summed) HIP_OK(launch_chain(a, s));
        h->owed.tail_summed = false;
        if (!h->xchg.on) { rc = allreduce_hook(h, s); if (rc) return rc; }
    }
    HIP_OK(hipMemcpyAsync(h->thermo.d_state + h->thermo.L.off_ke, h->thermo.d_state + h->thermo.L.off_ke_red, sizeof(double) * h->thermo.L.NT,
                          hipMemcpyDeviceToDevice, s));
    return TGNH_OK;
}

static void drain_events(tgnh_handle h) {
    for (size_t i = 0; i < h->timing.ev_used; i++) {
        auto& e = h->timing.ev_pool[i];
        if (hipEventSynchronize(e.b) != hipSuccess) continue;
        float ms = 0;
        if (hipEventElapsedTime(&ms, e.a, e.b) == hipSuccess) { h->timing.t_total[e.kid] += ms; h->timing.t_count[e.kid] += 1; }
    }
    h->timing.ev_used = 0;
}
extern "C" tgnh_status tgnh_timing_enable(tgnh_handle h, int on) {
    CHECK_H(h);
    if (h->host_only) return fail(TGNH_ERR_STATE, "host-only handle");
    HIP_OK(hipSetDevice(h->device));
    if (!on) drain_events(h);
    else {
        for (int k = 0; k < KID_COUNT; k++) { h->timing.t_total[k] = 0; h->timing.t_count[k] = 0; }
        h->timing.ev_used = 0;
        while (h->timing.ev_pool.size() < 2048) {
            tgnh_context::Timing::Ev e; e.kid = 0;
            if (hipEventCreate(&e.a) != hipSuccess) break;
            if (hipEventCreate(&e.b) != hipSuccess) { (void)hipEventDestroy(e.a); break; }
            h->timing.ev_pool.push_back(e);
        }
    }
    h->timing.on = on != 0;
    h->timing.only = on >= 2 ? on - 2 : -1;
    return TGNH_OK;
}
extern "C" tgnh_status tgnh_timing_read(tgnh_handle h, int kernel, double* total_ms, int64_t* launches) {
    CHECK_H(h);
    if (kernel < 0 || kernel >= KID_COUNT) return fail(TGNH_ERR_ARG, "bad kernel id");
    if (!h->host_only) { HIP_OK(hipSetDevice(h->device)); drain_events(h); }
    if (total_ms) *total_ms = h->timing.t_total[kernel];
    if (launches) *launches = h->timing.t_count[kernel];
    return TGNH_OK;
}
extern "C" tgnh_status tgnh_algorithmic_bytes(tgnh_handle h, int kernel, double* bytes) {
    CHECK_H(h);
    if (!bytes) return fail(TGNH_ERR_ARG, "null out");
    const double N = h->d.num_particles;
    const double V = h->d.precision == TGNH_PREC_SINGLE ? 16 : 32;
    const double F = 24;
    const double X = h->d.precision == TGNH_PREC_SINGLE ? 16 : 32;
    double b = 0;
    switch (kernel) {
        case KID_SKD: b = N * (2 * V + F + 2 * X); break;
        case KID_KICK_KE: b = N * (V + F); break;
        case KID_SCALE: b = N * (2 * V + (h->owed.end_folded ? F : 0)); break;
        case KID_KE: b = N * V; break;
        case KID_FORCE: b = N * (X + F); break;
        case KID_STEP:
            b = (h->d.flags & TGNH_FLAG_DEFER_SCALE) ? N * (3 * V + 2 * F + 2 * X) : N * (6 * V + 3 * F + 2 * X) / 2; break;
        default: b = 0;
    }
    *bytes = b;
    return TGNH_OK;
}
```

### openmm_drudenose_amd/csrc/tgnh_step.cpp

```cpp
#include "tgnh_host.h"

constexpr int64_t STATUS_POLL_EVERY = 64;

void note_status(tgnh_handle h, uint32_t flags) {
    if (h->status.failed_code) return;
    if (flags & 8u) {
        h->status.failed_code = TGNH_ERR_STATE;
        h->status.failed = "resident step (noticed at step " + std::to_string((long long)h->run.step_count) + "): the launch's work-groups did "
                    "not all become resident within the time limit (TGNH_FLAG_RESIDENT_STEP needs the device to itself)";
        if (flags & 4u) h->status.failed += "; the waiting work-groups timed out in turn (status bits 2 and 3)";
    } else if (flags & 16u) {
        h->status.failed_code = TGNH_ERR_STATE;
        h->status.failed = "kinetic-energy pass (noticed at step " + std::to_string((long long)h->run.step_count) + "): work-group 0 did not "
                    "receive every work-group's row of sums within the time limit (the sums were left as NaN: nothing integrated "
                    "on with a partial sum); the device is shared with something that keeps this launch's work-groups from running "
                    "-- or a chain was handed a NaN kinetic energy: with an all-reduce attached, the rank on which that happened";
    } else if (flags & 4u) {
        h->status.failed_code = TGNH_ERR_STATE;
        h->status.failed = "mailbox exchange timed out (noticed at step " + std::to_string((long long)h->run.step_count) +
                    "): a peer did not send its kinetic-energy sums; the run cannot continue";
    } else if ((flags & 1u) && h->d.mode == TGNH_MODE_DUALNH) {
        h->status.failed_code = TGNH_ERR_HARDWALL;
        h->status.failed = "Drude particle moved too far beyond hard wall constraint";
    }
}

static tgnh_status need_buffers(tgnh_handle h) {
    if (h->host_only) return fail(TGNH_ERR_STATE, "host-only handle (device -1): no GPU work can be launched on it");
    if (!h->bound.velm) return fail(TGNH_ERR_STATE, "tgnh_bind_buffers has not been called");
    return TGNH_OK;
}

static bool rescale_sums_rows(tgnh_handle h, int rows) {
    return h->cfg.inline_chain && !h->xchg.on && !h->xchg.allreduce && h->thermo.L.NT <= CHAIN_INLINE_SUM_NT &&
           (rows + h->topo.num_big <= h->cfg.inline_sum_rows || h->cfg.inline_sum_all);
}
static bool ke_carries(tgnh_handle h) { return h->cfg.carry_ok && !h->xchg.allreduce && !h->xchg.on; }
static bool big_com_on(tgnh_handle h) { return h->topo.num_big && com_thermostat_on(h->d); }
tgnh_status allreduce_hook(tgnh_handle h, hipStream_t s) {
    if (h->xchg.allreduce && h->xchg.allreduce(h->thermo.d_state + h->thermo.L.off_ke_red, h->thermo.L.NT, (void*)s, h->xchg.allreduce_user) != 0)
        return fail(TGNH_ERR_HIP, "all-reduce hook failed");
    return TGNH_OK;
}
static tgnh_status timed_chain(tgnh_handle h, const ChainArgs& a, hipStream_t s) { Timed t(h, s, KID_CHAIN); HIP_OK(launch_chain(a, s)); return TGNH_OK; }

template <typename Args> static Args common_args(tgnh_handle h, const double* scale) {
    Args a{};
    a.posq = h->bound.posq; a.posq_corr = h->bound.posq_corr; a.velm = h->bound.velm;
    a.force = reinterpret_cast<const long long*>(h->bound.force); a.pos_delta = h->bound.pos_delta;
    a.scale = scale ? scale : h->thermo.d_state + h->thermo.L.off_scale;
    a.partials = h->thermo.d_partials; a.status = h->status.d_word;
    a.padded = h->d.padded_num_particles;
    a.use_com = com_thermostat_on(h->d) ? 1 : 0;
    a.hardwall = h->d.max_drude_distance > 0 ? 1 : 0;
    a.dt = h->d.step_size; a.max_dist = h->d.max_drude_distance;
    a.hw_scale = std::sqrt(h->d.kB * h->d.drude_temperature);
    return a;
}

static TileArgs tile_args(tgnh_handle h, const double* scale) {
    TileArgs a = common_args<TileArgs>(h, scale);
    a.meta = h->topo.d_meta; a.tile_start = h->topo.d_tile_start; a.tile_res = h->topo.d_tile_res; a.res_table = h->topo.d_res_table;
    a.big_com = h->topo.d_big_com;
    a.num_tiles = h->topo.num_tiles; a.num_groups = h->thermo.L.G;
    a.reverse = h->run.sweep_reverse;
    a.wave_tile = h->topo.d_wave_tile; a.wmeta = h->topo.d_wmeta; a.num_wtiles = h->topo.num_wtiles;
    a.tile_pat = h->topo.d_tile_pat; a.pattern = h->topo.d_pattern; a.wpattern = h->topo.d_wpattern;
    return a;
}

static int grid_for(tgnh_handle h, int ops, bool hardwall, size_t lds) {
    if (h->cfg.grid_override > 0) return std::min(h->topo.num_tiles, h->cfg.grid_override);
    const int key = ops | (hardwall ? 1 << 16 : 0);
    auto it = h->cfg.grid_cache.find(key);
    if (it != h->cfg.grid_cache.end()) return it->second;
    int per_cu = tile_blocks_per_cu(h->d.precision, ops, h->cfg.gb, lds, (ops & OP_SCALE) && h->cfg.inline_chain && h->thermo.L.C > 1);
    if (per_cu < 1) per_cu = 2;
    int g = std::min(std::min(h->topo.num_tiles, per_cu * h->cfg.num_cus), GRID_CAP);
    if (g < 1) g = 1;
    h->cfg.grid_cache[key] = g;
    return g;
}

static int wave_grid_for(tgnh_handle h, int ops) {
    const int nw = h->topo.num_wtiles, need = (nw + TBLOCK / 64 - 1) / (TBLOCK / 64);
    if (h->cfg.grid_override > 0) return std::max(1, std::min(need, h->cfg.grid_override));
    const int key = ops | (1 << 17);
    auto it = h->cfg.grid_cache.find(key);
    if (it != h->cfg.grid_cache.end()) return it->second;
    int per_cu = wke_blocks_per_cu(h->d.precision, ops, h->cfg.gb);
    if (per_cu < 1) per_cu = 2;
#ifdef TGNH_TUNING
    if (const char* e = getenv("TGNH_WKE_PER_CU")) { int v = atoi(e); if (v >= 1) per_cu = std::min(per_cu, v); }
#endif
    int g = std::max(1, std::min(std::min(need, per_cu * h->cfg.num_cus), GRID_CAP));
    h->cfg.grid_cache[key] = g;
    return g;
}

static tgnh_status commit_stage(tgnh_handle h, hipStream_t s);

static size_t tagged_words_allocated() { return (size_t)2 * GRID_CAP * CHAIN_INLINE_SUM_NT; }
static size_t tagged_words_touched(int grid, int NT) {
    if (grid < 1) return 0;
    const int r = grid - 1, j = 2 * NT - 1;
    return ((size_t)(r >> 6) * (2 * CHAIN_INLINE_SUM_NT) + j) * 64 + (r & 63) + 1;
}

static tgnh_status check_launch(tgnh_handle h, const TileArgs& a, int grid, int block, bool wave, bool tagged) {
    if (grid < 1 || grid > GRID_CAP || grid > h->cfg.grid) return fail(TGNH_ERR_STATE, "internal: grid exceeds the partial-row table");
    if (wave) {
        if (!a.wave_tile || (int)h->topo.wave_tile.size() != a.num_wtiles + 1 || a.num_wtiles < 1)
            return fail(TGNH_ERR_STATE, "internal: wave-tile table does not match the launch");
        if ((long long)grid * (block / 64) > (long long)a.num_wtiles + (block / 64) - 1)
            return fail(TGNH_ERR_STATE, "internal: more work-groups than wave tiles");
    } else if (grid > h->topo.num_tiles) return fail(TGNH_ERR_STATE, "internal: more work-groups than tiles");
    if (tagged) {
        if (!a.rows || !a.sync || h->thermo.L.NT > CHAIN_INLINE_SUM_NT || tagged_words_touched(grid, h->thermo.L.NT) > tagged_words_allocated())
            return fail(TGNH_ERR_STATE, "internal: tagged rows do not fit their area");
    }
    return TGNH_OK;
}

extern "C" tgnh_status tgnh_get_launch_bounds(tgnh_handle h, int32_t out[8]) {
    CHECK_H(h);
    if (!out) return fail(TGNH_ERR_ARG, "null out");
    const int nw = h->topo.num_wtiles;
    int g = h->topo.num_tiles;
    if (nw > 0) g = std::max(g, (nw + TBLOCK / 64 - 1) / (TBLOCK / 64));
    g = std::max(1, std::min(g, GRID_CAP));
    const bool tagged = h->thermo.L.NT <= CHAIN_INLINE_SUM_NT && (h->meet.d_rows != nullptr || h->host_only);
    out[0] = h->topo.num_tiles; out[1] = nw; out[2] = (int)h->topo.wave_tile.size(); out[3] = g;
    out[4] = h->cfg.grid; out[5] = tagged ? (int)tagged_words_allocated() : 0;
    out[6] = tagged ? (int)tagged_words_touched(g, h->thermo.L.NT) : 0; out[7] = h->thermo.L.NT;
    return TGNH_OK;
}

static tgnh_status run_big_com(tgnh_handle h, bool kick, hipStream_t s) {
    BigComArgs b{};
    b.table = h->topo.d_big_table; b.n = h->topo.num_big; b.velm = h->bound.velm;
    b.force = reinterpret_cast<const long long*>(h->bound.force); b.padded = h->d.padded_num_particles;
    b.kick = kick ? 1 : 0; b.dt = h->d.step_size;
    b.big_com = h->topo.d_big_com;
    b.partials = h->thermo.d_partials + (size_t)GRID_CAP * h->thermo.L.NT; b.NT = h->thermo.L.NT; b.G = h->thermo.L.G;
    Timed t(h, s, KID_OTHER);
    HIP_OK(launch_big_com(h->d.precision, b, s));
    return TGNH_OK;
}

GatherArgs gather_args(tgnh_handle h, const double* scale) {
    GatherArgs a = common_args<GatherArgs>(h, scale);
    a.group = h->gather.d_group; a.resid = h->gather.d_resid;
    a.res_table = h->gather.d_res_table; a.partner = h->gather.d_partner; a.com = h->gather.d_com;
    a.n = h->d.num_particles;
    a.com_lanes = h->gather.com_lanes;
    a.n_res = a.use_com ? (int)h->gather.res_table.size() : 0;
    a.G = h->thermo.L.G; a.NT = h->thermo.L.NT;
    return a;
}

static tgnh_status run_gather(tgnh_handle h, int ops, int kid, hipStream_t s, const double* scale) {
    GatherArgs a = gather_args(h, scale);
    if ((ops & (OP_POSDELTA | OP_MOVE)) && !h->bound.pos_delta) return fail(TGNH_ERR_STATE, "posDelta buffer not bound");
    const int upd = ops & (OP_SCALE | OP_KICK | OP_DRIFT | OP_POSDELTA | OP_MOVE | OP_PREKICK);
    if (ops & OP_NOSTORE) return fail(TGNH_ERR_STATE, "internal: the gather path stores every kick");
    Timed t(h, s, kid);
    if (upd) {
        if ((upd & OP_SCALE) && a.use_com && !(h->owed.g_com_fresh && !(upd & OP_PREKICK))) {
            a.kick_com = (upd & OP_PREKICK) ? 1 : 0;
            HIP_OK(launch_gather_com(h->d.precision, a, s));
        }
        h->owed.g_com_fresh = false;
        a.ops = upd;
        HIP_OK(launch_gather_update(h->d.precision, a, s));
    }
    if (ops & OP_KE) {
        a.kick_com = 0;
        if (a.use_com) HIP_OK(launch_gather_com(h->d.precision, a, s));
        const int grid = gather_ke_grid(a);
        HIP_OK(launch_gather_ke(h->d.precision, a, grid, s));
        h->run.ke_parts = grid;
        h->owed.tail_summed = false;
        h->owed.g_com_fresh = a.use_com != 0;
    }
    return TGNH_OK;
}

tgnh_status run_chain_gather(tgnh_handle h, hipStream_t s, bool sum_only) {
    ChainArgs a = chain_args(h);
    Timed t(h, s, KID_CHAIN);
    HIP_OK(launch_gather_rowsum(h->thermo.d_partials, h->run.ke_parts, h->thermo.L.NT, h->thermo.d_state + h->thermo.L.off_ke_red, s));
    { tgnh_status rc = allreduce_hook(h, s); if (rc) return rc; }
    if (!sum_only) HIP_OK(launch_gather_chain(a, h->gather.d_scratch, s));
    return TGNH_OK;
}

static tgnh_status adopt_chain(tgnh_handle h, TileArgs& a, hipStream_t s) {
    const bool pingpong = h->owed.carry_pending && h->owed.stage_pending;
    if (h->owed.stage_pending && !pingpong) { tgnh_status rc = commit_stage(h, s); if (rc) return rc; }
    a.chain_on = 1;
    a.chain = chain_args(h);
    a.chain.chain_twice = h->owed.chain_pending_twice ? 1 : 0;
    a.chain.ke_carry = h->owed.carry_pending ? 1 : 0;
    a.sum_rows = h->owed.sum_pending ? (h->run.ke_parts + h->topo.num_big <= h->cfg.inline_sum_rows ? 1 : 2) : 0;
    a.x_wait = h->owed.xwait_pending ? 1 : 0;
    a.st_in = pingpong ? h->thermo.d_stage : h->thermo.d_state;
    a.st_out = pingpong ? h->thermo.d_state : h->thermo.d_stage;
    return TGNH_OK;
}

static tgnh_status ke_pass_prologue(tgnh_handle h, TileArgs& a, int ops, bool wave, int grid, hipStream_t s) {
    if (h->owed.stage_pending && !a.chain_on) {
        a.commit_len = h->thermo.L.total; a.commit_src = h->thermo.d_stage; a.commit_dst = h->thermo.d_state;
        a.commit_skip = h->thermo.L.off_ke_red; a.commit_skip_n = h->thermo.L.NT;
        h->owed.stage_pending = false;
    }
    h->owed.tail_summed = wave && h->meet.d_rows && !h->xchg.on && h->thermo.L.NT <= CHAIN_INLINE_SUM_NT && !rescale_sums_rows(h, grid);
    if (h->owed.tail_summed) { a.tail_sum = 1; a.rows = h->meet.d_rows; a.sync = h->meet.d_sync; a.ke_red = h->thermo.d_state + h->thermo.L.off_ke_red; }
    h->run.ke_parts = grid;
    return big_com_on(h) ? run_big_com(h, (ops & OP_KICK) != 0, s) : TGNH_OK;
}

static tgnh_status launch_pass(tgnh_handle h, int ops, int kid, const TileArgs& a, bool wave, int grid, size_t lds, hipStream_t s) {
    tgnh_status rc = check_launch(h, a, grid, TBLOCK, wave, a.tail_sum != 0); if (rc) return rc;
    Timed t(h, s, kid);
    if (wave) HIP_OK(launch_wke(h->d.precision, ops, h->cfg.gb, a, grid, s));
    else HIP_OK(launch_tile(h->d.precision, ops, h->cfg.gb, a, grid, lds, s));
    return TGNH_OK;
}

tgnh_status run_tile(tgnh_handle h, int ops, int kid, hipStream_t s, const double* scale) {
    if (h->gather.generic) return run_gather(h, ops, kid, s, scale);
    tgnh_status rc;
    TileArgs a = tile_args(h, scale);
    if ((ops & OP_SCALE) && h->owed.chain_pending && !scale) { rc = adopt_chain(h, a, s); if (rc) return rc; }
    if ((ops & (OP_POSDELTA | OP_MOVE)) && !h->bound.pos_delta) return fail(TGNH_ERR_STATE, "posDelta buffer not bound");
    size_t lds = tile_lds_bytes(h->d.precision, ops, a.hardwall != 0, a.use_com != 0);
    if ((ops & OP_KE) && h->cfg.gb == 0) lds += sizeof(double) * (TBLOCK / 64) * h->thermo.L.G;
    const bool wave = h->cfg.wave_ke && (ops & OP_KE) && !(ops & ~(OP_KE | OP_KICK | OP_NOSTORE));
    const int grid = wave ? wave_grid_for(h, ops) : grid_for(h, ops, a.hardwall != 0, lds);
    if (ops & OP_KE) { rc = ke_pass_prologue(h, a, ops, wave, grid, s); if (rc) return rc; }
    rc = launch_pass(h, ops, kid, a, wave, grid, lds, s); if (rc) return rc;
    if (a.chain_on) { h->owed.chain_ran(); h->owed.stage_pending = a.st_out == h->thermo.d_stage; }
    if (h->cfg.alternate_sweeps) h->run.sweep_reverse ^= 1;
    return TGNH_OK;
}

ChainArgs chain_args(tgnh_handle h) {
    ChainArgs a{};
    a.L = h->thermo.L; a.st = h->thermo.d_state; a.partials = h->thermo.d_partials; a.nparts = h->run.ke_parts;
    a.nbig = h->topo.num_big;
    a.dt = h->d.step_size; a.S = h->d.drude_steps_per_real_step;
    a.dtc = a.dt / a.S; a.inv_dtc = 1.0 / a.dtc;
    a.realkbT = h->thermo.realkbT; a.drudekbT = h->thermo.drudekbT;
#ifdef TGNH_TUNING
    if (const char* e = getenv("TGNH_CHAIN_LANES")) a.lanes = e[0] != '0';
#endif
    a.stage = h->thermo.d_stage;
    a.status = h->status.d_word;
    if (h->xchg.on) a.x = h->xchg.args;
    a.commit = h->owed.stage_pending ? 1 : 0;
    h->owed.stage_pending = false;
    return a;
}

static tgnh_status commit_stage(tgnh_handle h, hipStream_t s) {
    if (!h->owed.stage_pending) return TGNH_OK;
    ChainArgs a = chain_args(h);
    a.do_sum = 0; a.do_chain = 0;
    HIP_OK(launch_chain(a, s));
    return TGNH_OK;
}

static tgnh_status run_chain(tgnh_handle h, hipStream_t s, bool twice) {
    if (h->gather.chain) return run_chain_gather(h, s, false);
    const bool sum_next = rescale_sums_rows(h, h->run.ke_parts), sum_now = !sum_next && !h->owed.tail_summed;
    const bool mailbox = h->xchg.on, hook = !mailbox && h->xchg.allreduce;
    const bool chain_next = h->cfg.inline_chain;
    const bool chain_with_sum = !chain_next && !hook, chain_alone = !chain_next && hook;
    h->owed.tail_summed = false;
    tgnh_status rc;
    ChainArgs a = chain_args(h);
    a.chain_twice = twice ? 1 : 0;
    if (sum_now || chain_with_sum) {
        a.do_sum = sum_now ? 1 : 0; a.x_send = mailbox ? 1 : 0;
        a.do_chain = chain_with_sum ? 1 : 0; a.x_wait = mailbox && chain_with_sum ? 1 : 0;
        rc = timed_chain(h, a, s); if (rc) return rc;
    }
    if (hook) { rc = allreduce_hook(h, s); if (rc) return rc; }
    if (chain_alone) {
        a.do_sum = 0; a.do_chain = 1; a.commit = 0;
        rc = timed_chain(h, a, s); if (rc) return rc;
    }
    if (chain_next) { h->owed.chain_owed(twice); h->owed.sum_pending |= sum_next; h->owed.xwait_pending |= mailbox; }
    return TGNH_OK;
}

tgnh_status materialize_chain(tgnh_handle h, hipStream_t s) {
    { tgnh_status rc = settle_end(h, s); if (rc) return rc; }
    if (!h->owed.chain_pending) return commit_stage(h, s);
    ChainArgs a = chain_args(h);
    a.do_sum = h->owed.sum_pending ? 1 : 0; a.do_chain = 1; a.chain_twice = h->owed.chain_pending_twice ? 1 : 0;
    a.x_wait = h->owed.xwait_pending ? 1 : 0;
    a.ke_carry = h->owed.carry_pending ? 1 : 0;
    { tgnh_status rc = timed_chain(h, a, s); if (rc) return rc; }
    h->owed.chain_ran();
    return TGNH_OK;
}

static int resident_kernel(tgnh_handle h, int kind) {
    if (!((h->d.flags & TGNH_FLAG_RESIDENT_STEP) && h->cfg.inline_chain && h->cfg.gb != 0 && h->thermo.L.NT <= CHAIN_INLINE_SUM_NT &&
          (h->xchg.on || !h->xchg.allreduce))) return 0;
    if (kind == 0 && h->cfg.wresident_per_cu > 0) return 2;
    return h->cfg.resident_per_cu > 0 && h->thermo.L.C == 1 ? 1 : 0;
}
bool resident_now(tgnh_handle h) { return resident_kernel(h, pass_kind(h->d)) != 0; }

extern "C" tgnh_status tgnh_get_step_path(tgnh_handle h, int* gather, const char** reason) {
    CHECK_H(h);
    if (gather) *gather = h->gather.generic ? (h->gather.chain ? 2 : 1) : 0;
    if (reason) *reason = h->gather.reason.c_str();
    return TGNH_OK;
}

extern "C" tgnh_status tgnh_get_resident_kernel(tgnh_handle h, int* which) {
    CHECK_H(h);
    if (!which) return fail(TGNH_ERR_ARG, "null out");
    *which = resident_kernel(h, pass_kind(h->d));
    return TGNH_OK;
}

static tgnh_status run_resident(tgnh_handle h, hipStream_t s, int kind) {
    if (h->owed.stage_pending) { tgnh_status rc = commit_stage(h, s); if (rc) return rc; }
    TileArgs a = tile_args(h, nullptr);
    const int ops2 = step_kind_ops2(kind);
    if ((ops2 & OP_POSDELTA) && !h->bound.pos_delta) return fail(TGNH_ERR_STATE, "posDelta buffer not bound");
    const bool hw = a.hardwall != 0 && (ops2 & (OP_DRIFT | OP_MOVE));
    const size_t lds = tile_lds_bytes(h->d.precision, ops2, hw, a.use_com != 0);
    const bool wstep = resident_kernel(h, kind) == 2;
    int& grid = h->cfg.resident_grid[kind][hw ? 1 : 0];
    if (grid == 0 && !wstep) {
        int per_cu = std::min(h->cfg.resident_per_cu, step_blocks_per_cu(h->d.precision, h->cfg.gb, kind, lds));
        if (per_cu < 1) return fail(TGNH_ERR_HIP, "step_kernel: occupancy query failed");
        grid = std::max(1, std::min(std::min(h->topo.num_tiles, per_cu * h->cfg.num_cus / h->cfg.resident_share), GRID_CAP));
    }
    a.chain_on = 1;
    a.chain = chain_args(h);
    a.chain.chain_twice = kind == 0 ? 1 : 0;
    a.x_wait = 1;
    if (!h->xchg.on) a.chain.x = h->meet.self_x;
    a.st_in = h->thermo.d_state; a.st_out = h->thermo.d_state;
    a.sync = h->meet.d_sync; a.rows = h->meet.d_rows;
    if (big_com_on(h)) { tgnh_status rc = run_big_com(h, kind == 0 || kind == 2, s); if (rc) return rc; }
    if (wstep && h->cfg.wresident_grid == 0) {
        const int need = (h->topo.num_wtiles + WBLOCK / 64 - 1) / (WBLOCK / 64);
        h->cfg.wresident_grid = std::max(1, std::min(std::min(need, h->cfg.wresident_per_cu * h->cfg.num_cus / h->cfg.resident_share), GRID_CAP));
    }
    const int g = wstep ? h->cfg.wresident_grid : grid;
    a.chain.nparts = g;
    h->run.ke_parts = g;
    { tgnh_status rc = check_launch(h, a, g, wstep ? WBLOCK : TBLOCK, wstep, true); if (rc) return rc; }
    {
        Timed t(h, s, KID_STEP);
        if (wstep) HIP_OK(launch_wstep(h->d.precision, h->cfg.gb, h->thermo.L.C > 1, a, g, s));
        else HIP_OK(launch_step(h->d.precision, h->cfg.gb, kind, a, g, lds, s));
    }
    h->owed.resident_settled();
    return TGNH_OK;
}

static tgnh_status first_half(tgnh_handle h, hipStream_t s) {
    if (h->owed.first_half_done) return TGNH_OK;
    if (h->owed.ke_carry) {
        h->owed.ke_carry = false;
        if (big_com_on(h)) { tgnh_status rc = run_big_com(h, false, s); if (rc) return rc; }
        if (h->cfg.inline_chain) {
            h->owed.chain_owed(false); h->owed.sum_pending = false; h->owed.carry_pending = true;
            return TGNH_OK;
        }
        ChainArgs a = chain_args(h);
        a.do_sum = 0; a.do_chain = 1; a.ke_carry = 1;
        return timed_chain(h, a, s);
    }
    tgnh_status rc = run_tile(h, OP_KE, KID_KE, s); if (rc) return rc;
    return run_chain(h, s, false);
}

tgnh_status entry(tgnh_handle h, bool need_bufs) {
    if (!h) return fail(TGNH_ERR_ARG, "null handle");
    h->owed.g_com_fresh = false;
    if (need_bufs) { tgnh_status rc = need_buffers(h); if (rc) return rc; }
    if (!h->host_only) {
        HIP_OK(hipSetDevice(h->device));
        if (h->status.h_seen) note_status(h, *h->status.h_seen);
    }
    if (h->status.failed_code) return fail(h->status.failed_code, h->status.failed);
    return TGNH_OK;
}

static tgnh_status poll_status_async(tgnh_handle h, hipStream_t s) {
    if (!h->status.h_seen || h->run.step_count % STATUS_POLL_EVERY != 0) return TGNH_OK;
    hipStreamCaptureStatus cs = hipStreamCaptureStatusNone;
    if (s != nullptr && hipStreamIsCapturing(s, &cs) == hipSuccess && cs != hipStreamCaptureStatusNone) return TGNH_OK;
    HIP_OK(hipMemcpyAsync(h->status.h_seen, h->status.d_word, sizeof(uint32_t), hipMemcpyDeviceToHost, s));
    return TGNH_OK;
}

static void start_of_step(tgnh_handle h) {
    if (h->cfg.alternate_sweeps) h->run.sweep_reverse = (int)(h->run.step_count & 1);
}
static tgnh_status advance_clock(tgnh_handle h, hipStream_t s) {
    h->run.time += h->d.step_size; h->run.step_count += 1;
    return poll_status_async(h, s);
}

extern "C" tgnh_status tgnh_step_begin(tgnh_handle h, void* stream) {
    tgnh_status rc = entry(h, true); if (rc) return rc;
    hipStream_t s = (hipStream_t)stream;
    start_of_step(h);
    if (h->owed.end_pending) {
        if (resident_now(h)) return run_resident(h, s, 0);
        rc = settle_end(h, s); if (rc) return rc;
    }
    if (!(h->d.flags & TGNH_FLAG_DEFER_SCALE) && resident_now(h) && !h->owed.ke_carry)
        return run_resident(h, s, 1);
    rc = first_half(h, s); if (rc) return rc;
    rc = run_tile(h, (h->owed.kick_pending ? OP_PREKICK : 0) | OP_SCALE | OP_KICK | OP_DRIFT, KID_SKD, s); if (rc) return rc;
    h->owed.velocities_current(); h->owed.first_half_done = false;
    return TGNH_OK;
}

static tgnh_status second_half(tgnh_handle h, hipStream_t s, int kick_ops) {
    tgnh_status rc;
    const bool defer = (h->d.flags & TGNH_FLAG_DEFER_SCALE) != 0;
    h->owed.ke_carry = false;
    if (h->owed.scale_pending || h->owed.kick_pending || h->owed.end_pending) { rc = flush_impl(h, s); if (rc) return rc; }
    if (!defer && resident_now(h)) {
        rc = run_resident(h, s, kick_ops ? 2 : 4); if (rc) return rc;
        h->owed.ke_carry = ke_carries(h);
    } else if (kick_ops && resident_now(h)) {
        h->owed.end_pending = true;
    } else {
        const bool fold = !defer && kick_ops != 0 && !h->gather.generic;
        const int nostore = kick_ops && !h->gather.generic ? OP_NOSTORE : 0;
        h->owed.end_folded = fold;
        rc = run_tile(h, kick_ops | OP_KE | nostore, kick_ops ? KID_KICK_KE : KID_KE, s); if (rc) return rc;
        rc = run_chain(h, s, defer); if (rc) return rc;
        if (defer) h->owed.end_half_deferred(nostore != 0);
        else {
            rc = run_tile(h, (fold ? OP_PREKICK : 0) | OP_SCALE, KID_SCALE, s); if (rc) return rc;
            h->owed.ke_carry = ke_carries(h);
        }
    }
    return advance_clock(h, s);
}

extern "C" tgnh_status tgnh_step_end(tgnh_handle h, void* stream) {
    tgnh_status rc = entry(h, true); if (rc) return rc;
    return second_half(h, (hipStream_t)stream, OP_KICK);
}

tgnh_status settle_kick(tgnh_handle h, hipStream_t s) {
    return (h->owed.kick_pending || h->owed.end_pending) ? flush_impl(h, s) : TGNH_OK;
}

tgnh_status settle_end(tgnh_handle h, hipStream_t s) {
    if (!h->owed.end_pending) return TGNH_OK;
    h->owed.end_pending = false;
    tgnh_status rc = run_tile(h, OP_KICK | OP_KE | OP_NOSTORE, KID_KICK_KE, s); if (rc) return rc;
    rc = run_chain(h, s, true); if (rc) return rc;
    h->owed.end_half_deferred(true);
    return TGNH_OK;
}

static tgnh_status split_entry(tgnh_handle h, hipStream_t s, bool fresh_ke) {
    tgnh_status rc = entry(h, true); if (rc) return rc;
    if (fresh_ke) h->owed.ke_carry = false;
    return settle_kick(h, s);
}

extern "C" tgnh_status tgnh_step_begin_kick(tgnh_handle h, void* stream) {
    hipStream_t s = (hipStream_t)stream;
    tgnh_status rc = split_entry(h, s, false); if (rc) return rc;
    start_of_step(h);
    if (!(h->d.flags & TGNH_FLAG_DEFER_SCALE) && resident_now(h) && !h->owed.ke_carry) return run_resident(h, s, 3);
    rc = first_half(h, s); if (rc) return rc;
    rc = run_tile(h, OP_SCALE | OP_KICK | OP_POSDELTA, KID_OTHER, s); if (rc) return rc;
    h->owed.scale_pending = false; h->owed.first_half_done = false;
    return TGNH_OK;
}
extern "C" tgnh_status tgnh_step_begin_move(tgnh_handle h, void* stream) {
    tgnh_status rc = split_entry(h, (hipStream_t)stream, true); if (rc) return rc;
    return run_tile(h, OP_MOVE, KID_OTHER, (hipStream_t)stream);
}
extern "C" tgnh_status tgnh_step_end_kick(tgnh_handle h, void* stream) {
    tgnh_status rc = split_entry(h, (hipStream_t)stream, true); if (rc) return rc;
    return run_tile(h, OP_KICK, KID_OTHER, (hipStream_t)stream);
}
extern "C" tgnh_status tgnh_step_end_thermo(tgnh_handle h, void* stream) {
    tgnh_status rc = entry(h, true); if (rc) return rc;
    return second_half(h, (hipStream_t)stream, 0);
}
extern "C" tgnh_status tgnh_half_kick(tgnh_handle h, void* stream) { return tgnh_step_end_kick(h, stream); }

tgnh_status flush_impl(tgnh_handle h, hipStream_t s) {
    tgnh_status rc = settle_end(h, s); if (rc) return rc;
    if (!h->owed.scale_pending && !h->owed.kick_pending) return TGNH_OK;
    rc = materialize_chain(h, s); if (rc) return rc;
    if (h->owed.scale_pending) {
        rc = run_tile(h, (h->owed.kick_pending ? OP_PREKICK : 0) | OP_SCALE, KID_SCALE, s, h->thermo.d_state + h->thermo.L.off_scale_a); if (rc) return rc;
        HIP_OK(hipMemcpyAsync(h->thermo.d_state + h->thermo.L.off_scale, h->thermo.d_state + h->thermo.L.off_scale_b, sizeof(double) * h->thermo.L.NT,
                              hipMemcpyDeviceToDevice, s));
    } else {
        rc = run_tile(h, OP_KICK, KID_OTHER, s); if (rc) return rc;
    }
    if (big_com_on(h)) { rc = run_big_com(h, false, s); if (rc) return rc; }
    h->owed.velocities_current();
    return TGNH_OK;
}

extern "C" tgnh_status tgnh_flush(tgnh_handle h, void* stream) {
    CHECK_H(h);
    if (!h->owed.scale_pending && !h->owed.kick_pending && !h->owed.end_pending) return TGNH_OK;
    tgnh_status rc = entry(h, true); if (rc) return rc;
    return flush_impl(h, (hipStream_t)stream);
}

extern "C" tgnh_status tgnh_note_replayed_steps(tgnh_handle h, int nsteps) {
    CHECK_H(h);
    if (nsteps < 0) return fail(TGNH_ERR_ARG, "negative step count");
    h->run.time += h->d.step_size * nsteps;
    h->run.step_count += nsteps;
    return TGNH_OK;
}

extern "C" tgnh_status tgnh_set_time(tgnh_handle h, double time, int64_t step_count) {
    CHECK_H(h);
    if (step_count < 0) return fail(TGNH_ERR_ARG, "negative step count");
    h->run.time = time;
    h->run.step_count = step_count;
    return TGNH_OK;
}

extern "C" tgnh_status tgnh_get_pending_state(tgnh_handle h, uint32_t* bits) {
    CHECK_H(h);
    if (!bits) return fail(TGNH_ERR_ARG, "null out");
    *bits = h->owed.bits() | (h->run.sweep_reverse ? (uint32_t)tgnh_context::Owed::BIT_SWEEP_REVERSE : 0u);
    return TGNH_OK;
}

extern "C" tgnh_status tgnh_state_changed(tgnh_handle h) {
    CHECK_H(h);
    tgnh_status rc = deferred_guard(h, "tgnh_state_changed");
    if (rc) return rc;
    h->owed.ke_carry = false;
    return TGNH_OK;
}
```

### openmm_drudenose_amd/drudetgnhplugin.py

```python
import ctypes as C

import numpy as np

from . import _lib
from ._lib import (MODE_DUALNH, MODE_TGNH, PREC_SINGLE, PREC_MIXED, PREC_DOUBLE,
                   FLAG_DEFER_SCALE, FLAG_RESIDENT_STEP, FLAG_WAVE_TILES, FLAG_TRUST_STATE_CHANGED, FLAG_GATHER)
from .synth import KB

_PREC = {"single": PREC_SINGLE, "mixed": PREC_MIXED, "double": PREC_DOUBLE}
_MODE = {"dualNH": MODE_DUALNH, "TGNH": MODE_TGNH}


class TgnhError(RuntimeError):

    def __init__(self, status, message):
        super().__init__(message)
        self.status = status


def _check(rc):
    if rc != _lib.TGNH_OK:
        raise TgnhError(rc, _lib.load().tgnh_last_error().decode())


class DrudeTGNHIntegrator:

    def __init__(self, temperature, couplingTime, drudeTemperature, drudeCouplingTime, stepSize,
                 drudeStepsPerRealStep=20, numNHChains=1, useDrudeNHChains=True, useCOMTempGroup=True):
        self._temperature = float(temperature)
        self._couplingTime = float(couplingTime)
        self._drudeTemperature = float(drudeTemperature)
        self._drudeCouplingTime = float(drudeCouplingTime)
        self._maxDrudeDistance = 0.0
        self._stepSize = float(stepSize)
        self._drudeSteps = int(drudeStepsPerRealStep)
        self._numNHChains = int(numNHChains)
        self._useDrudeNHChains = bool(useDrudeNHChains)
        self._useCOMTempGroup = bool(useCOMTempGroup)
        self._constraintTolerance = 1e-5
        self._tempGroups = []
        self._particleTempGroup = []
        self._context = None

    def getTemperature(self): return self._temperature
    def setTemperature(self, temp): self._temperature = float(temp)
    def getCouplingTime(self): return self._couplingTime
    def setCouplingTime(self, tau): self._couplingTime = float(tau)
    def getDrudeTemperature(self): return self._drudeTemperature
    def setDrudeTemperature(self, temp): self._drudeTemperature = float(temp)
    def getDrudeCouplingTime(self): return self._drudeCouplingTime
    def setDrudeCouplingTime(self, tau): self._drudeCouplingTime = float(tau)
    def getMaxDrudeDistance(self): return self._maxDrudeDistance

    def setMaxDrudeDistance(self, distance):
        if distance < 0:
            raise TgnhError(_lib.ERR_ARG, "setMaxDrudeDistance: Distance cannot be negative")
        self._maxDrudeDistance = float(distance)
        if self._context is not None:
            self._context._push_scalars()

    def getStepSize(self): return self._stepSize

    def setStepSize(self, dt):
        self._stepSize = float(dt)
        if self._context is not None:
            self._context._push_scalars()

    def getConstraintTolerance(self): return self._constraintTolerance
    def setConstraintTolerance(self, tol): self._constraintTolerance = float(tol)
    def getDrudeStepsPerRealStep(self): return self._drudeSteps

    def setDrudeStepsPerRealStep(self, drudeSteps):
        self._drudeSteps = int(drudeSteps)
        if self._context is not None:
            self._context._push_scalars()

    def getNumNHChains(self): return self._numNHChains
    def setNumNHChains(self, numChains): self._numNHChains = int(numChains)
    def getUseDrudeNHChains(self): return int(self._useDrudeNHChains)
    def setUseDrudeNHChains(self, use): self._useDrudeNHChains = bool(use)
    def getUseCOMTempGroup(self): return int(self._useCOMTempGroup)
    def setUseCOMTempGroup(self, use): self._useCOMTempGroup = bool(use)

    def getNumTempGroups(self): return len(self._tempGroups)

    def addTempGroup(self):
        self._tempGroups.append(len(self._tempGroups))
        return len(self._tempGroups) - 1

    def addParticleTempGroup(self, tempGroup):
        if not 0 <= tempGroup < len(self._tempGroups):
            raise TgnhError(_lib.ERR_ARG, "Index out of range")
        if not isinstance(self._particleTempGroup, list):
            self._particleTempGroup = [int(x) for x in self._particleTempGroup]
        self._particleTempGroup.append(int(tempGroup))
        return len(self._particleTempGroup) - 1

    def setParticleTempGroup(self, particle, tempGroup):
        if not 0 <= particle < len(self._particleTempGroup) or not 0 <= tempGroup < len(self._tempGroups):
            raise TgnhError(_lib.ERR_ARG, "Index out of range")
        self._particleTempGroup[particle] = int(tempGroup)

    def getParticleTempGroup(self, particle):
        if not 0 <= particle < len(self._particleTempGroup):
            raise TgnhError(_lib.ERR_ARG, "Index out of range")
        return int(self._particleTempGroup[particle])

    def step(self, steps):
        if self._context is None:
            raise TgnhError(_lib.ERR_STATE, "This Integrator is not bound to a context!")
        self._context.step(steps)

    def computeKineticEnergy(self):
        return self._context.kinetic_energy()

    def _resolve_groups(self, num_particles):
        if len(self._particleTempGroup) == 0:
            if len(self._tempGroups) == 0:
                self._tempGroups.append(0)
            self._particleTempGroup = np.zeros(num_particles, np.int32)
        elif len(self._particleTempGroup) != num_particles:
            raise TgnhError(_lib.ERR_ARG, "Number of particles assigned with temperature groups does not match the number of system particles")
        return np.asarray(self._particleTempGroup, np.int32), len(self._tempGroups)


def create_handle(lib, system, integrator, group, ngroups, mode, precision, device, flags, kB, padded):
    n = system.num_particles
    d = _lib.TgnhDesc()
    d.struct_size = C.sizeof(_lib.TgnhDesc)
    d.mode, d.precision, d.flags, d.device = mode, precision, int(flags), device
    d.num_particles, d.padded_num_particles = n, padded
    d.num_pairs, d.num_groups, d.num_residues = system.num_pairs, ngroups, system.num_residues
    d.num_constraints = len(system.constraints)
    d.has_cm_motion_remover = int(system.has_cm_motion_remover)
    group = np.ascontiguousarray(group, np.int32)
    ci = np.ascontiguousarray(system.constraints[:, 0]) if len(system.constraints) else None
    cj = np.ascontiguousarray(system.constraints[:, 1]) if len(system.constraints) else None
    d.mass = system.mass.ctypes.data_as(_lib.c_f64p)
    d.pair_drude = system.pair_drude.ctypes.data_as(_lib.c_i32p)
    d.pair_parent = system.pair_parent.ctypes.data_as(_lib.c_i32p)
    d.group = group.ctypes.data_as(_lib.c_i32p)
    d.resid = system.resid.ctypes.data_as(_lib.c_i32p)
    if ci is not None:
        d.constraint_i = ci.ctypes.data_as(_lib.c_i32p)
        d.constraint_j = cj.ctypes.data_as(_lib.c_i32p)
    d.kB = kB
    d.temperature, d.coupling_time = integrator.getTemperature(), integrator.getCouplingTime()
    d.drude_temperature, d.drude_coupling_time = integrator.getDrudeTemperature(), integrator.getDrudeCouplingTime()
    d.step_size = integrator.getStepSize()
    d.drude_steps_per_real_step = integrator.getDrudeStepsPerRealStep()
    d.num_nh_chains = integrator.getNumNHChains()
    d.use_drude_nh_chains = integrator.getUseDrudeNHChains()
    d.use_com_temp_group = integrator.getUseCOMTempGroup()
    d.max_drude_distance = integrator.getMaxDrudeDistance()
    h = C.c_void_p()
    _check(lib.tgnh_create(C.byref(d), C.byref(h)))
    return h


class _HandleQueries:

    def _stream(self):
        return None

    def step_path(self):
        g, why = C.c_int(), C.c_char_p()
        _check(self.lib.tgnh_get_step_path(self.h, C.byref(g), C.byref(why)))
        return ("tiled", "gather", "gather")[g.value], (why.value or b"").decode()

    def local_dof_terms(self):
        n = C.c_int()
        _check(self.lib.tgnh_get_local_dof_terms(self.h, None, C.byref(n)))
        out = np.zeros(n.value)
        _check(self.lib.tgnh_get_local_dof_terms(self.h, out.ctypes.data_as(_lib.c_f64p), C.byref(n)))
        return out

    def set_global_dof_terms(self, total):
        total = np.ascontiguousarray(total, np.float64)
        _check(self.lib.tgnh_set_global_dof_terms(self.h, total.ctypes.data_as(_lib.c_f64p), len(total)))

    def num_thermostats(self):
        n = C.c_int()
        _check(self.lib.tgnh_get_num_thermostats(self.h, C.byref(n)))
        return n.value

    def dof(self):
        n = self.num_thermostats()
        dof, nkt = np.zeros(n), np.zeros(n)
        _check(self.lib.tgnh_get_dof(self.h, dof.ctypes.data_as(_lib.c_f64p), nkt.ctypes.data_as(_lib.c_f64p)))
        return dof, nkt

    def thermostat_state(self, which):
        n = C.c_int()
        _check(self.lib.tgnh_get_thermostat_len(self.h, which, C.byref(n)))
        out = np.zeros(n.value)
        _check(self.lib.tgnh_get_thermostat_state(self.h, which, self._stream(), out.ctypes.data_as(_lib.c_f64p)))
        return out

    def set_thermostat_state(self, which, arr):
        arr = np.ascontiguousarray(arr, np.float64)
        _check(self.lib.tgnh_set_thermostat_state(self.h, which, self._stream(), arr.ctypes.data_as(_lib.c_f64p)))

    def topology(self, which):
        n = C.c_int()
        _check(self.lib.tgnh_get_topology_len(self.h, which, C.byref(n)))
        out = np.zeros(n.value, np.int32)
        _check(self.lib.tgnh_get_topology(self.h, which, out.ctypes.data_as(_lib.c_i32p)))
        return out


class HostTopology(_HandleQueries):

    def __init__(self, system, integrator, mode="TGNH", precision="mixed", flags=0, kB=KB):
        self.lib = _lib.load()
        group, ngroups = integrator._resolve_groups(system.num_particles)
        self.group, self.num_groups = group, ngroups
        n = system.num_particles
        self.h = create_handle(self.lib, system, integrator, group, ngroups, _MODE[mode], _PREC[precision], -1, flags, kB,
                               (n + 31) // 32 * 32)

    def close(self):
        if getattr(self, "h", None):
            self.lib.tgnh_destroy(self.h)
            self.h = None

    def __del__(self):
        try:
            self.close()
        except Exception:
            pass


class HipContext(_HandleQueries):

    def __init__(self, system, integrator, mode="TGNH", precision="mixed", device=0, flags=0, kB=KB,
                 k_drude=None, k_tether=None, allreduce=None, global_dof_sum=None, lattice_sites=True):
        import torch
        self.torch = torch
        self.lib = _lib.load()
        if not torch.cuda.is_available():
            raise RuntimeError("the DrudeTGNH HIP path needs a GPU (torch.cuda.is_available() is False); there is no CPU fallback")
        self.system, self.integrator = system, integrator
        self.mode, self.precision = _MODE[mode], _PREC[precision]
        self.dev = torch.device("cuda", device)
        n = system.num_particles
        self.n = n
        self.padded = (n + 31) // 32 * 32
        group, ngroups = integrator._resolve_groups(n)
        self.group, self.num_groups = group, ngroups
        from .synth import K_DRUDE, K_TETHER
        self.k_drude = K_DRUDE if k_drude is None else k_drude
        self.k_tether = K_TETHER if k_tether is None else k_tether

        with torch.cuda.device(self.dev):
            h = create_handle(self.lib, system, integrator, group, ngroups, self.mode, self.precision, device, flags, kB,
                              self.padded)
        self.h = h
        self._hook = None
        if global_dof_sum is not None:
            self.set_global_dof_terms(global_dof_sum(self.local_dof_terms()))
        if allreduce is not None:
            self.set_allreduce(allreduce)

        rdt = torch.float32 if self.precision != PREC_DOUBLE else torch.float64
        mdt = torch.float32 if self.precision == PREC_SINGLE else torch.float64
        self.rdt, self.mdt = rdt, mdt
        self.posq = torch.zeros((n, 4), dtype=rdt, device=self.dev)
        self.posq_corr = torch.zeros((n, 4), dtype=torch.float32, device=self.dev) if self.precision == PREC_MIXED else None
        self.velm = torch.zeros((n, 4), dtype=mdt, device=self.dev)
        self.force = torch.zeros(3 * self.padded, dtype=torch.int64, device=self.dev)
        self.pos_delta = torch.zeros((n, 4), dtype=mdt, device=self.dev)
        self.x0 = torch.zeros((n, 4), dtype=rdt, device=self.dev)
        self.sites_packed = False
        self.unpacked_sites = False
        self.use_lattice_sites = bool(lattice_sites)
        inv = np.where(system.mass == 0.0, 0.0, 1.0 / np.where(system.mass == 0.0, 1.0, system.mass))
        self.velm[:, 3] = torch.from_numpy(inv).to(self.dev, mdt)
        _check(self.lib.tgnh_bind_buffers(self.h, self.posq.data_ptr(),
                                          self.posq_corr.data_ptr() if self.posq_corr is not None else None,
                                          self.velm.data_ptr(), self.force.data_ptr(), self.pos_delta.data_ptr()))
        integrator._context = self
        self.force_fn = None
        self.state_hook = None
        self.ke_sum_valid = False
        self.constrained = False
        if system.cluster_atoms is not None and len(system.cluster_atoms):
            _check(self.lib.tgnh_harness_set_clusters(self.h, len(system.cluster_atoms),
                                                      system.cluster_atoms.ctypes.data_as(_lib.c_i32p),
                                                      system.cluster_dist.ctypes.data_as(_lib.c_f64p)))
            self.constrained = True
        if system.site_atoms is not None and len(system.site_atoms):
            _check(self.lib.tgnh_harness_set_virtual_sites(self.h, len(system.site_atoms),
                                                           system.site_atoms.ctypes.data_as(_lib.c_i32p),
                                                           system.site_weights.ctypes.data_as(_lib.c_f64p)))
            self.constrained = True
        if system.positions is not None:
            self.setPositions(system.positions)
            self.set_sites(system.positions)
        if system.velocities is not None:
            self.setVelocities(system.velocities)
        if system.positions is not None:
            self.compute_forces()

    def _stream(self):
        return C.c_void_p(self.torch.cuda.current_stream(self.dev).cuda_stream)

    def _push_scalars(self):
        i = self.integrator
        _check(self.lib.tgnh_set_step_size(self.h, i.getStepSize()))
        _check(self.lib.tgnh_set_drude_steps_per_real_step(self.h, i.getDrudeStepsPerRealStep()))
        _check(self.lib.tgnh_set_max_drude_distance(self.h, i.getMaxDrudeDistance()))

    def close(self):
        if getattr(self, "h", None):
            self.torch.cuda.synchronize(self.dev)
            self.lib.tgnh_destroy(self.h)
            self.h = None

    def __del__(self):
        try:
            self.close()
        except Exception:
            pass

    def set_allreduce(self, fn):
        torch = self.torch

        def _hook(buf, count, stream, user):
            try:
                t = self._ke_view(buf, count)
                fn(t)
                return 0
            except Exception as e:
                print("all-reduce hook failed:", e)
                return 1
        self._hook = _lib.ALLREDUCE_FN(_hook)
        self._views = {}
        _check(self.lib.tgnh_set_allreduce(self.h, self._hook, None))

    RCCL_ID_BYTES = 128

    def rccl_init(self, world, rank, unique_id):
        _check(self.lib.tgnh_rccl_init(self.h, int(world), int(rank), C.c_char_p(unique_id)))
        self._hook = None

    def rccl_unique_id(self):
        buf = C.create_string_buffer(self.RCCL_ID_BYTES)
        _check(self.lib.tgnh_rccl_unique_id(buf))
        return buf.raw

    def rccl_shutdown(self):
        _check(self.lib.tgnh_rccl_shutdown(self.h))

    def rccl_init_over(self, dist, rank, world):
        ok, err = 1, None
        ids = [None]
        try:
            mine = self.rccl_unique_id()
            if rank == 0:
                ids[0] = mine
        except Exception as e:
            ok, err = 0, e
        votes = [None] * world
        dist.all_gather_object(votes, ok)
        if not all(votes):
            self.rccl_error = err or RuntimeError("RCCL could not be bound on rank(s) " + str([r for r, v in enumerate(votes) if not v]))
            return False
        dist.broadcast_object_list(ids, src=0)
        try:
            self.rccl_init(world, rank, ids[0])
        except Exception as e:
            ok, err = 0, e
        flags = [None] * world
        dist.all_gather_object(flags, ok)
        if not all(flags):
            if ok:
                self.rccl_shutdown()
            self.rccl_error = err
            return False
        return True

    XCHG_HANDLE_BYTES = 64

    def exchange_wait_stats(self):
        mean, mx, n = C.c_double(), C.c_double(), C.c_int64()
        _check(self.lib.tgnh_exchange_wait_stats(self.h, self._stream(), C.byref(mean), C.byref(mx), C.byref(n)))
        return mean.value, mx.value, n.value

    def exchange_create(self, world, rank):
        buf = C.create_string_buffer(self.XCHG_HANDLE_BYTES)
        ptr = C.c_void_p()
        _check(self.lib.tgnh_exchange_create(self.h, int(world), int(rank), buf, C.byref(ptr)))
        return buf.raw, ptr.value

    def exchange_attach(self, handles):
        blob = b"".join(handles)
        _check(self.lib.tgnh_exchange_attach(self.h, blob))

    def exchange_attach_pointers(self, pointers):
        arr = (C.c_void_p * len(pointers))(*[C.c_void_p(p) for p in pointers])
        _check(self.lib.tgnh_exchange_attach_pointers(self.h, arr))

    def set_resident_share(self, share):
        _check(self.lib.tgnh_set_resident_share(self.h, int(share)))

    def resident_work_groups(self):
        n = C.c_int()
        _check(self.lib.tgnh_get_resident_work_groups(self.h, C.byref(n)))
        return n.value

    def resident_kernel(self):
        n = C.c_int()
        _check(self.lib.tgnh_get_resident_kernel(self.h, C.byref(n)))
        return (None, "step_kernel", "wstep_kernel")[n.value]

    def exchange_detach(self):
        _check(self.lib.tgnh_exchange_detach(self.h))

    def attach_exchange_over(self, dist, rank, world, tensor_device="cuda"):
        torch = self.torch
        ok, err = 1, None
        try:
            handle, _ = self.exchange_create(world, rank)
            handles = [None] * world
            dist.all_gather_object(handles, handle)
            self.exchange_attach(handles)
        except Exception as e:
            ok, err = 0, e
        t = torch.tensor([ok], dtype=torch.int32, device=tensor_device)
        dist.all_reduce(t, op=dist.ReduceOp.MIN)
        if int(t.item()) == 0:
            if ok:
                self.exchange_detach()
            self.exchange_error = err
            return False
        return True

    def _ke_view(self, ptr, count):
        key = (ptr, count)
        v = self._views.get(key)
        if v is None:
            torch = self.torch

            class _Holder:
                pass
            hold = _Holder()
            hold.__cuda_array_interface__ = {"shape": (count,), "typestr": "<f8", "data": (ptr, False), "version": 2}
            v = torch.as_tensor(hold, device=self.dev)
            self._views[key] = v
        return v

    def setPositions(self, pos):
        torch = self.torch
        self._state_changed()
        p = torch.from_numpy(np.ascontiguousarray(pos, np.float64)).to(self.dev)
        if self.precision == PREC_DOUBLE:
            self.posq[:, :3] = p
        else:
            hi = p.to(torch.float32)
            self.posq[:, :3] = hi
            if self.posq_corr is not None:
                self.posq_corr[:, :3] = (p - hi.to(torch.float64)).to(torch.float32)

    def set_sites(self, x0):
        self.x0[:, :3] = self.torch.from_numpy(np.ascontiguousarray(x0, np.float64)).to(self.dev, self.rdt)
        flag = (self.system.mass > 0)
        flag[self.system.pair_drude] = False
        self.x0[:, 3] = self.torch.from_numpy(flag.astype(np.float64)).to(self.dev, self.rdt)
        self.torch.cuda.synchronize(self.dev)
        lat = getattr(self.system, "lattice", None)
        if lat is not None and self.use_lattice_sites:
            k, side, spacing, geom, first = lat
            geom = np.ascontiguousarray(geom, np.float64)
            _check(self.lib.tgnh_harness_lattice_hint(self.h, int(k), int(side), float(spacing), geom.ctypes.data_as(_lib.c_f64p), int(first)))
        else:
            _check(self.lib.tgnh_harness_lattice_hint(self.h, 0, 0, 0.0, None, 0))
        _check(self.lib.tgnh_harness_pack_sites(self.h, self.x0.data_ptr()))
        self.sites_packed = True

    def sites_kind(self):
        n = C.c_int()
        _check(self.lib.tgnh_harness_sites_kind(self.h, C.byref(n)))
        return ("x0", "packed", "lattice")[n.value]

    def _x0_arg(self):
        return None if self.sites_packed and not self.unpacked_sites else self.x0.data_ptr()

    def sites(self):
        return self.x0[:, :3].to(self.torch.float64).cpu().numpy()

    def setVelocities(self, vel):
        self._state_changed()
        self.velm[:, :3] = self.torch.from_numpy(np.ascontiguousarray(vel, np.float64)).to(self.dev, self.mdt)

    def _state_changed(self):
        self.ke_sum_valid = False
        _check(self.lib.tgnh_state_changed(self.h))

    def getPositions(self):
        p = self.posq[:, :3].to(self.torch.float64)
        if self.posq_corr is not None:
            p = p + self.posq_corr[:, :3].to(self.torch.float64)
        return p.cpu().numpy()

    def flush(self):
        _check(self.lib.tgnh_flush(self.h, self._stream()))

    def getVelocities(self):
        _check(self.lib.tgnh_flush(self.h, self._stream()))
        return self.velm[:, :3].to(self.torch.float64).cpu().numpy()

    def getForces(self):
        f = self.force.view(3, self.padded)[:, :self.n].to(self.torch.float64) / 4294967296.0
        return f.t().contiguous().cpu().numpy()

    def setForces(self, f):
        t = self.torch.from_numpy(np.ascontiguousarray(f, np.float64)).to(self.dev)
        self.force.view(3, self.padded)[:, :self.n] = (t * 4294967296.0).to(self.torch.int64).t()

    def compute_forces(self):
        if self.force_fn is not None:
            self.force_fn(self)
        else:
            _check(self.lib.tgnh_harness_force(self.h, self._x0_arg(), self.k_drude, self.k_tether,
                                               self.force.data_ptr(), self._stream()))

    def step_begin(self):
        _check(self.lib.tgnh_step_begin(self.h, self._stream()))

    def step_end(self):
        _check(self.lib.tgnh_step_end(self.h, self._stream()))
        self.ke_sum_valid = True

    def step(self, steps):
        if self.force_fn is None and self.constrained:
            _check(self.lib.tgnh_run_harness_constrained(self.h, self._x0_arg(), self.k_drude, self.k_tether,
                                                         self.integrator.getConstraintTolerance(), int(steps), self._stream()))
            if steps > 0:
                self.ke_sum_valid = True
            return
        if self.force_fn is None:
            _check(self.lib.tgnh_run_harness(self.h, self._x0_arg(), self.k_drude, self.k_tether, int(steps), self._stream()))
            if steps > 0:
                self.ke_sum_valid = True
            return
        lib, h = self.lib, self.h
        for _ in range(steps):
            if self.state_hook is not None:
                self.state_hook(self)
            if not self.constrained:
                self.step_begin()
                self.compute_forces()
                self.step_end()
                continue
            tol = self.integrator.getConstraintTolerance()
            _check(lib.tgnh_step_begin_kick(h, self._stream()))
            _check(lib.tgnh_harness_shake_positions(h, tol, self._stream()))
            _check(lib.tgnh_step_begin_move(h, self._stream()))
            _check(lib.tgnh_harness_virtual_sites(h, self._stream()))
            self.compute_forces()
            _check(lib.tgnh_step_end_kick(h, self._stream()))
            if self.mode == MODE_TGNH:
                _check(lib.tgnh_harness_shake_velocities(h, tol, self._stream()))
            _check(lib.tgnh_step_end_thermo(h, self._stream()))
            self.ke_sum_valid = True

    def step_without_forces(self, steps):
        if self.constrained:
            raise TgnhError(_lib.ERR_STATE, "step_without_forces: unconstrained systems only")
        _check(self.lib.tgnh_run_steps(self.h, int(steps), self._stream()))
        if steps > 0:
            self.ke_sum_valid = True

    def capture_steps(self, steps, forces=True):
        torch = self.torch
        if self.force_fn is not None:
            raise TgnhError(_lib.ERR_STATE, "capture_steps supports the harness force call-out only")
        torch.cuda.synchronize(self.dev)
        def record():
            g = torch.cuda.CUDAGraph()
            with torch.cuda.graph(g):
                if self.constrained and not forces:
                    raise TgnhError(_lib.ERR_STATE, "capture_steps(forces=False): unconstrained systems only")
                if self.constrained:
                    _check(self.lib.tgnh_run_harness_constrained(self.h, self._x0_arg(), self.k_drude, self.k_tether,
                                                                 self.integrator.getConstraintTolerance(), int(steps), self._stream()))
                elif not forces:
                    _check(self.lib.tgnh_run_steps(self.h, int(steps), self._stream()))
                else:
                    _check(self.lib.tgnh_run_harness(self.h, self._x0_arg(), self.k_drude, self.k_tether, int(steps), self._stream()))
            return g
        for _ in range(4):
            owed_before = self.pending_state() & 0x2ff
            first = record()
            if self.pending_state() & 0x2ff == owed_before:
                break
            first.replay()
            torch.cuda.synchronize(self.dev)
            self.ke_sum_valid = True
        else:
            raise TgnhError(_lib.ERR_STATE, "capture_steps: the handle does not reach a steady state of its step sequence")
        clock = self.time()
        graphs = [first, record()]
        if self.pending_state() & 0x2ff != owed_before:
            raise TgnhError(_lib.ERR_STATE, "capture_steps: the step sequence is not periodic")
        self.set_time(*clock)
        self._captured_not_run = int(steps)
        turn = [0]

        def replay():
            graphs[turn[0] & 1].replay()
            turn[0] += 1
            if self._captured_not_run:
                self._captured_not_run = 0
            else:
                _check(self.lib.tgnh_note_replayed_steps(self.h, int(steps)))
            self.ke_sum_valid = True
        replay.graph = graphs[0]
        replay.graphs = graphs
        return replay

    def pending_state(self):
        bits = C.c_uint32()
        _check(self.lib.tgnh_get_pending_state(self.h, C.byref(bits)))
        return bits.value

    def status_flags(self):
        flags = C.c_uint32()
        self.lib.tgnh_get_status_flags(self.h, self._stream(), C.byref(flags))
        return flags.value

    def check(self):
        flags = C.c_uint32()
        _check(self.lib.tgnh_get_status_flags(self.h, self._stream(), C.byref(flags)))
        return flags.value

    def _vec(self, fn, n):
        out = np.zeros(n)
        _check(fn(self.h, self._stream(), out.ctypes.data_as(_lib.c_f64p)))
        return out

    def last_kinetic_energies(self):
        return self._vec(self.lib.tgnh_get_last_kinetic_energies, self.num_thermostats())

    def last_scale_factors(self):
        return self._vec(self.lib.tgnh_get_last_scale_factors, self.num_thermostats())

    def compute_kinetic_energies(self):
        _check(self.lib.tgnh_compute_kinetic_energies(self.h, self._stream()))
        return self.last_kinetic_energies()

    def half_kick(self):
        _check(self.lib.tgnh_half_kick(self.h, self._stream()))

    def kinetic_energy(self):
        out = C.c_double()
        _check(self.lib.tgnh_get_kinetic_energy(self.h, int(self.ke_sum_valid), self._stream(), C.byref(out)))
        return out.value

    def time(self):
        t, k = C.c_double(), C.c_int64()
        _check(self.lib.tgnh_get_time(self.h, C.byref(t), C.byref(k)))
        return t.value, k.value

    def set_time(self, time, step_count):
        _check(self.lib.tgnh_set_time(self.h, float(time), int(step_count)))

    def timing(self, on):
        _check(self.lib.tgnh_timing_enable(self.h, int(on)))

    def timing_read(self, kid):
        ms, n = C.c_double(), C.c_int64()
        _check(self.lib.tgnh_timing_read(self.h, kid, C.byref(ms), C.byref(n)))
        return ms.value, n.value

    def algorithmic_bytes(self, kid):
        b = C.c_double()
        _check(self.lib.tgnh_algorithmic_bytes(self.h, kid, C.byref(b)))
        return b.value
```

Measured before the change: 4078 steps/s.

## Capture K-step integrator loops into HIP graphs and replay them in run loops

run_steps and run_harness now go through a shared run_loop. When the loop is long enough and no exchange, timing, gather path or capture is active, it records two K-step HIP graphs, one per step parity, and replays them instead of launching each kernel eagerly. Host-side owed/run state is restored after recording and advanced per replay. Every setter that changes launch arguments invalidates the held graphs. This targets per-step host launch and dispatch overhead, at the cost of recording time, extra state bookkeeping, and an eager fallback when the state is not periodic.

```diff
diff --git a/include/drude_tgnh.h b/include/drude_tgnh.h
--- a/include/drude_tgnh.h
+++ b/include/drude_tgnh.h
@@ -34,6 +34,8 @@
 enum { TGNH_FLAG_TRUST_STATE_CHANGED = 16 };
 
 enum { TGNH_FLAG_GATHER = 32 };
+
+enum { TGNH_FLAG_EAGER_LOOPS = 64 };
 
 typedef struct tgnh_desc {
     uint32_t struct_size;
@@ -144,6 +146,8 @@
 tgnh_status tgnh_run_steps(tgnh_handle h, int nsteps, void* stream);
 tgnh_status tgnh_run_harness(tgnh_handle h, const void* x0, double k_drude, double k_tether,
                              int nsteps, void* stream);
+tgnh_status tgnh_replay_probe(tgnh_handle h, int nsteps, void* stream, int32_t out[6]);
+tgnh_status tgnh_set_replay_steps(tgnh_handle h, int steps_per_graph);
 
 tgnh_status tgnh_harness_set_clusters(tgnh_handle h, int n, const int32_t* atoms, const double* dist);
 tgnh_status tgnh_harness_shake_positions(tgnh_handle h, double tol, void* stream);
diff --git a/openmm_drudenose_amd/_lib.py b/openmm_drudenose_amd/_lib.py
--- a/openmm_drudenose_amd/_lib.py
+++ b/openmm_drudenose_amd/_lib.py
@@ -8,7 +8,7 @@
 ERR_ARG, ERR_GROUP_MISMATCH, ERR_HARDWALL, ERR_UNSUPPORTED, ERR_HIP, ERR_STATE = -1, -2, -3, -4, -5, -6
 MODE_DUALNH, MODE_TGNH = 0, 1
 PREC_SINGLE, PREC_MIXED, PREC_DOUBLE = 0, 1, 2
-FLAG_DEFER_SCALE, FLAG_RESIDENT_STEP, FLAG_WAVE_TILES, FLAG_TRUST_STATE_CHANGED, FLAG_GATHER = 2, 4, 8, 16, 32
+FLAG_DEFER_SCALE, FLAG_RESIDENT_STEP, FLAG_WAVE_TILES, FLAG_TRUST_STATE_CHANGED, FLAG_GATHER, FLAG_EAGER_LOOPS = 2, 4, 8, 16, 32, 64
 KID_SKD, KID_KICK_KE, KID_SCALE, KID_KE, KID_CHAIN, KID_FORCE, KID_OTHER, KID_STEP = range(8)
 KERNEL_NAMES = {KID_SKD: "scale+kick+drift", KID_KICK_KE: "kick+KE", KID_SCALE: "rescale", KID_KE: "KE",
                 KID_CHAIN: "chain", KID_FORCE: "harness force", KID_OTHER: "other", KID_STEP: "resident step"}
@@ -92,6 +92,8 @@
     "tgnh_harness_sites_kind": (C.c_int, [C.c_void_p, C.POINTER(C.c_int)]),
     "tgnh_run_harness": (C.c_int, [C.c_void_p, C.c_void_p, C.c_double, C.c_double, C.c_int, C.c_void_p]),
     "tgnh_run_steps": (C.c_int, [C.c_void_p, C.c_int, C.c_void_p]),
+    "tgnh_replay_probe": (C.c_int, [C.c_void_p, C.c_int, C.c_void_p, c_i32p]),
+    "tgnh_set_replay_steps": (C.c_int, [C.c_void_p, C.c_int]),
     "tgnh_harness_set_clusters": (C.c_int, [C.c_void_p, C.c_int, c_i32p, c_f64p]),
     "tgnh_harness_shake_positions": (C.c_int, [C.c_void_p, C.c_double, C.c_void_p]),
     "tgnh_harness_shake_velocities": (C.c_int, [C.c_void_p, C.c_double, C.c_void_p]),
diff --git a/openmm_drudenose_amd/csrc/tgnh_context.h b/openmm_drudenose_amd/csrc/tgnh_context.h
--- a/openmm_drudenose_amd/csrc/tgnh_context.h
+++ b/openmm_drudenose_amd/csrc/tgnh_context.h
@@ -36,6 +36,27 @@
     operator T*() const { return p_; }
 };
 typedef DeviceBuf<unsigned char> DeviceBytes;
+class GraphExec {
+    hipGraphExec_t g_ = nullptr;
+public:
+    GraphExec() = default;
+    GraphExec(const GraphExec&) = delete;
+    GraphExec& operator=(const GraphExec&) = delete;
+    ~GraphExec() { reset(); }
+    void reset() { if (g_) (void)hipGraphExecDestroy(g_); g_ = nullptr; }
+    hipError_t instantiate(hipGraph_t g) { reset(); return hipGraphInstantiate(&g_, g, nullptr, nullptr, 0); }
+    operator hipGraphExec_t() const { return g_; }
+};
+class OwnedStream {
+    hipStream_t s_ = nullptr;
+public:
+    OwnedStream() = default;
+    OwnedStream(const OwnedStream&) = delete;
+    OwnedStream& operator=(const OwnedStream&) = delete;
+    ~OwnedStream() { if (s_) (void)hipStreamDestroy(s_); }
+    hipError_t create() { return s_ ? hipSuccess : hipStreamCreateWithFlags(&s_, hipStreamNonBlocking); }
+    operator hipStream_t() const { return s_; }
+};
 }
 
 struct tgnh_context {
@@ -132,6 +153,26 @@
         int sweep_reverse = 0;
         int ke_parts = 0;
     } run;
+    struct Replay {
+        int K = 50;
+        tgnh::OwnedStream capture;
+        bool held = false;
+        struct Recording {
+            tgnh::GraphExec exec;
+            int parity = 0;
+            Owed owed_after;
+            int sweep_after = 0;
+        } rec[2];
+        uint32_t key = 0;
+        int ke_parts = 0;
+        bool forces = false;
+        const void* x0 = nullptr;
+        double k_drude = 0, k_tether = 0;
+        int failures = 0;
+        int64_t recordings = 0, launches = 0, eager_steps = 0;
+        const char* dropped_by = "";
+        void drop() { rec[0].exec.reset(); rec[1].exec.reset(); held = false; failures = 0; }
+    } replay;
     struct Bound {
         void *posq = nullptr, *posq_corr = nullptr, *velm = nullptr, *pos_delta = nullptr;
         const void* force = nullptr;
diff --git a/openmm_drudenose_amd/csrc/tgnh_exchange.cpp b/openmm_drudenose_amd/csrc/tgnh_exchange.cpp
--- a/openmm_drudenose_amd/csrc/tgnh_exchange.cpp
+++ b/openmm_drudenose_amd/csrc/tgnh_exchange.cpp
@@ -46,6 +46,7 @@
     h->xchg.args.peers = h->xchg.d_peers; h->xchg.args.mine = h->xchg.mailbox; h->xchg.args.seq = h->xchg.d_seq; h->xchg.args.dead = h->xchg.d_dead;
     h->xchg.args.status = h->status.d_word;
     h->xchg.args.stat = h->xchg.d_stat;
+    replay_touched(h, TOUCH_EXCHANGE);
     h->xchg.on = true;
     return TGNH_OK;
 }
@@ -104,6 +105,7 @@
         HIP_OK(hipDeviceSynchronize());
     }
     h->xchg.on = false;
+    replay_touched(h, TOUCH_EXCHANGE);
     h->xchg.close_peers();
     return TGNH_OK;
 }
@@ -113,6 +115,7 @@
     tgnh_status rc = deferred_guard(h, "tgnh_set_allreduce"); if (rc) return rc;
     h->owed.ke_carry = false;
     if (h->xchg.rccl_comm) { rc = tgnh_rccl_shutdown(h); if (rc) return rc; }
+    if (fn != h->xchg.allreduce || user != h->xchg.allreduce_user) replay_touched(h, TOUCH_EXCHANGE);
     h->xchg.allreduce = fn; h->xchg.allreduce_user = user;
     return TGNH_OK;
 }
@@ -182,6 +185,7 @@
         if (h->xchg.allreduce == rccl_allreduce) { h->xchg.allreduce = nullptr; h->xchg.allreduce_user = nullptr; }
         return TGNH_OK;
     }
+    replay_touched(h, TOUCH_EXCHANGE);
     h->xchg.rccl_comm = nccl_comm; h->xchg.rccl_owned = false;
     h->xchg.allreduce = rccl_allreduce; h->xchg.allreduce_user = h;
     return TGNH_OK;
@@ -200,6 +204,7 @@
     std::memcpy(&uid, id, sizeof(uid));
     ncclComm_t comm = nullptr;
     RCCL_OK(rccl().CommInitRank(&comm, world, uid, rank));
+    replay_touched(h, TOUCH_EXCHANGE);
     h->xchg.rccl_comm = comm; h->xchg.rccl_owned = true;
     h->xchg.allreduce = rccl_allreduce; h->xchg.allreduce_user = h;
     return TGNH_OK;
@@ -213,6 +218,7 @@
     ncclComm_t comm = static_cast<ncclComm_t>(h->xchg.rccl_comm);
     const bool owned = h->xchg.rccl_owned;
     h->xchg.rccl_comm = nullptr; h->xchg.rccl_owned = false;
+    replay_touched(h, TOUCH_EXCHANGE);
     if (owned) RCCL_OK(rccl().CommDestroy(comm));
     return TGNH_OK;
 }
@@ -243,6 +249,7 @@
 extern "C" tgnh_status tgnh_set_resident_share(tgnh_handle h, int share) {
     CHECK_H(h);
     if (share < 1 || share > 64) return fail(TGNH_ERR_ARG, "resident share must be 1..64");
+    if (share != h->cfg.resident_share) replay_touched(h, TOUCH_RESIDENT_SHARE);
     h->cfg.resident_share = share;
     h->cfg.wresident_grid = 0;
     for (auto& g : h->cfg.resident_grid) g[0] = g[1] = 0;
diff --git a/openmm_drudenose_amd/csrc/tgnh_harness_host.cpp b/openmm_drudenose_amd/csrc/tgnh_harness_host.cpp
--- a/openmm_drudenose_amd/csrc/tgnh_harness_host.cpp
+++ b/openmm_drudenose_amd/csrc/tgnh_harness_host.cpp
@@ -32,6 +32,7 @@
     tgnh_status rc = entry(h, false); if (rc) return rc;
     if (h->host_only) return fail(TGNH_ERR_STATE, "host-only handle");
     if (!x0) return fail(TGNH_ERR_ARG, "null x0");
+    replay_touched(h, TOUCH_SITES);
     const int N = h->d.num_particles;
     const size_t rs = h->d.precision == TGNH_PREC_DOUBLE ? sizeof(double) : sizeof(float);
     if (h->gather.generic) {
@@ -94,6 +95,7 @@
 extern "C" tgnh_status tgnh_harness_lattice_hint(tgnh_handle h, int mol_slots, int side, double spacing, const double* geom, int first_molecule) {
     CHECK_H(h);
     h->harness.lat_on = false;
+    replay_touched(h, TOUCH_SITES);
     if (mol_slots == 0) { h->harness.lat_k = 0; h->harness.lat_geom.clear(); return TGNH_OK; }
     if (mol_slots < 1 || mol_slots > 64 || side < 1 || side > 1290 || !(spacing > 0) || !geom || first_molecule < 0) return fail(TGNH_ERR_ARG, "bad lattice hint");
     h->harness.lat_k = mol_slots; h->harness.lat_side = side; h->harness.lat_spacing = spacing; h->harness.lat_mol0 = first_molecule;
@@ -109,20 +111,9 @@
 
 extern "C" tgnh_status tgnh_run_harness(tgnh_handle h, const void* x0, double k_drude, double k_tether,
                                         int nsteps, void* stream) {
-    CHECK_H(h);
-    for (int i = 0; i < nsteps; i++) {
-        tgnh_status rc = tgnh_step_begin(h, stream); if (rc) return rc;
-        rc = tgnh_harness_force(h, x0, k_drude, k_tether, const_cast<void*>(h->bound.force), stream); if (rc) return rc;
-        rc = tgnh_step_end(h, stream); if (rc) return rc;
-    }
-    return TGNH_OK;
+    return run_loop(h, LoopCall{true, x0, k_drude, k_tether}, nsteps, stream);
 }
 
 extern "C" tgnh_status tgnh_run_steps(tgnh_handle h, int nsteps, void* stream) {
-    CHECK_H(h);
-    for (int i = 0; i < nsteps; i++) {
-        tgnh_status rc = tgnh_step_begin(h, stream); if (rc) return rc;
-        rc = tgnh_step_end(h, stream); if (rc) return rc;
-    }
-    return TGNH_OK;
+    return run_loop(h, LoopCall{false, nullptr, 0.0, 0.0}, nsteps, stream);
 }
diff --git a/openmm_drudenose_amd/csrc/tgnh_host.h b/openmm_drudenose_amd/csrc/tgnh_host.h
--- a/openmm_drudenose_amd/csrc/tgnh_host.h
+++ b/openmm_drudenose_amd/csrc/tgnh_host.h
@@ -38,6 +38,11 @@
 tgnh_status settle_kick(tgnh_handle h, hipStream_t s);
 tgnh_status settle_end(tgnh_handle h, hipStream_t s);
 tgnh_status flush_impl(tgnh_handle h, hipStream_t s);
+enum LoopTouch { TOUCH_BUFFERS, TOUCH_STEP_SIZE, TOUCH_DRUDE_STEPS, TOUCH_HARD_WALL, TOUCH_DOF_TERMS, TOUCH_THERMOSTAT_STATE, TOUCH_EXCHANGE,
+                 TOUCH_RESIDENT_SHARE, TOUCH_SITES, TOUCH_LOOP_ARGS, TOUCH_CLOCK, TOUCH_FAILURE, TOUCH_GRAPH_STEPS, TOUCH_COUNT };
+void replay_touched(tgnh_handle h, LoopTouch what);
+struct LoopCall { bool forces; const void* x0; double k_drude, k_tether; };
+tgnh_status run_loop(tgnh_handle h, const LoopCall& c, int nsteps, void* stream);
 
 struct Timed {
     tgnh_context* c; hipStream_t s; int kid; tgnh_context::Timing::Ev* ev = nullptr;
diff --git a/openmm_drudenose_amd/csrc/tgnh_lifecycle.cpp b/openmm_drudenose_amd/csrc/tgnh_lifecycle.cpp
--- a/openmm_drudenose_amd/csrc/tgnh_lifecycle.cpp
+++ b/openmm_drudenose_amd/csrc/tgnh_lifecycle.cpp
@@ -25,7 +25,7 @@
     if (d->mode == TGNH_MODE_TGNH && (d->num_groups < 1 || d->num_residues < 1 || !d->group || !d->resid))
         return fail(TGNH_ERR_ARG, "TGNH mode needs temperature groups and residues");
     if (!(d->max_drude_distance >= 0)) return fail(TGNH_ERR_ARG, "setMaxDrudeDistance: Distance cannot be negative");
-    if (d->flags & ~(uint32_t)(TGNH_FLAG_DEFER_SCALE | TGNH_FLAG_RESIDENT_STEP | TGNH_FLAG_WAVE_TILES | TGNH_FLAG_TRUST_STATE_CHANGED | TGNH_FLAG_GATHER))
+    if (d->flags & ~(uint32_t)(TGNH_FLAG_DEFER_SCALE | TGNH_FLAG_RESIDENT_STEP | TGNH_FLAG_WAVE_TILES | TGNH_FLAG_TRUST_STATE_CHANGED | TGNH_FLAG_GATHER | TGNH_FLAG_EAGER_LOOPS))
         return fail(TGNH_ERR_ARG, "unknown bits in tgnh_desc.flags (a newer header than this library?)");
     if (d->mode == TGNH_MODE_DUALNH && d->num_pairs == 0)
         return fail(TGNH_ERR_UNSUPPORTED, "dualNH mode needs at least one Drude pair (the Reference platform does too)");
@@ -229,6 +229,7 @@
         }
     }
     h->owed.ke_carry = false;
+    replay_touched(h, TOUCH_BUFFERS);
     h->bound.posq = posq; h->bound.posq_corr = posq_correction; h->bound.velm = velm; h->bound.force = force; h->bound.pos_delta = pos_delta;
     return TGNH_OK;
 }
@@ -243,6 +244,7 @@
     CHECK_H(h);
     if (!(dt > 0) || !std::isfinite(dt)) return fail(TGNH_ERR_ARG, "step size must be positive");
     if (dt != h->d.step_size) { tgnh_status rc = deferred_guard(h, "tgnh_set_step_size"); if (rc) return rc; }
+    if (dt != h->d.step_size) replay_touched(h, TOUCH_STEP_SIZE);
     h->d.step_size = dt;
     return TGNH_OK;
 }
@@ -250,12 +252,14 @@
     CHECK_H(h);
     if (n < 1) return fail(TGNH_ERR_ARG, "drudeStepsPerRealStep must be >= 1");
     if (n != h->d.drude_steps_per_real_step) { tgnh_status rc = deferred_guard(h, "tgnh_set_drude_steps_per_real_step"); if (rc) return rc; }
+    if (n != h->d.drude_steps_per_real_step) replay_touched(h, TOUCH_DRUDE_STEPS);
     h->d.drude_steps_per_real_step = n;
     return TGNH_OK;
 }
 extern "C" tgnh_status tgnh_set_max_drude_distance(tgnh_handle h, double dist) {
     CHECK_H(h);
     if (!(dist >= 0)) return fail(TGNH_ERR_ARG, "setMaxDrudeDistance: Distance cannot be negative");
+    if (dist != h->d.max_drude_distance) replay_touched(h, TOUCH_HARD_WALL);
     h->d.max_drude_distance = dist;
     return TGNH_OK;
 }
@@ -271,6 +275,7 @@
     if (!terms || count != h->thermo.L.NT) return fail(TGNH_ERR_ARG, "dof term count mismatch");
     if (h->run.step_count != 0) return fail(TGNH_ERR_STATE, "global dof must be set before the first step");
     if (!h->host_only) HIP_OK(hipSetDevice(h->device));
+    replay_touched(h, TOUCH_DOF_TERMS);
     h->thermo.global_terms.assign(terms, terms + count);
     return finalize_thermostat(h);
 }
diff --git a/openmm_drudenose_amd/csrc/tgnh_queries.cpp b/openmm_drudenose_amd/csrc/tgnh_queries.cpp
--- a/openmm_drudenose_amd/csrc/tgnh_queries.cpp
+++ b/openmm_drudenose_amd/csrc/tgnh_queries.cpp
@@ -96,6 +96,7 @@
     if (!in) return fail(TGNH_ERR_ARG, "null in");
     tgnh_status rc = deferred_guard(h, "tgnh_set_thermostat_state"); if (rc) return rc;
     h->owed.ke_carry = false;
+    replay_touched(h, TOUCH_THERMOSTAT_STATE);
     if (h->host_only) { std::copy(in, in + len, h->thermo.h_state.begin() + off); return TGNH_OK; }
     HIP_OK(hipSetDevice(h->device));
     rc = materialize_chain(h, (hipStream_t)stream); if (rc) return rc;
diff --git a/openmm_drudenose_amd/csrc/tgnh_step.cpp b/openmm_drudenose_amd/csrc/tgnh_step.cpp
--- a/openmm_drudenose_amd/csrc/tgnh_step.cpp
+++ b/openmm_drudenose_amd/csrc/tgnh_step.cpp
@@ -23,6 +23,7 @@
         h->status.failed_code = TGNH_ERR_HARDWALL;
         h->status.failed = "Drude particle moved too far beyond hard wall constraint";
     }
+    if (h->status.failed_code) replay_touched(h, TOUCH_FAILURE);
 }
 
 static tgnh_status need_buffers(tgnh_handle h) {
@@ -537,6 +538,7 @@
 extern "C" tgnh_status tgnh_set_time(tgnh_handle h, double time, int64_t step_count) {
     CHECK_H(h);
     if (step_count < 0) return fail(TGNH_ERR_ARG, "negative step count");
+    if (time != h->run.time || step_count != h->run.step_count) replay_touched(h, TOUCH_CLOCK);
     h->run.time = time;
     h->run.step_count = step_count;
     return TGNH_OK;
@@ -556,3 +558,148 @@
     h->owed.ke_carry = false;
     return TGNH_OK;
 }
+
+enum { LOOP_REPLAYS = 0, LOOP_EAGER_FLAG = 1, LOOP_EAGER_SHORT = 2, LOOP_EAGER_TIMING = 3, LOOP_EAGER_GATHER = 4, LOOP_EAGER_EXCHANGE = 5,
+       LOOP_EAGER_CAPTURING = 6, LOOP_EAGER_GAVE_UP = 7 };
+static int loop_verdict(tgnh_handle h, int nsteps, hipStream_t s) {
+    const struct { bool eager; int row; } table[] = {
+        {(h->d.flags & TGNH_FLAG_EAGER_LOOPS) != 0, LOOP_EAGER_FLAG},
+        {nsteps < 2 * h->replay.K, LOOP_EAGER_SHORT},
+        {h->timing.on, LOOP_EAGER_TIMING},
+        {h->gather.generic, LOOP_EAGER_GATHER},
+        {h->xchg.on || h->xchg.allreduce != nullptr || h->xchg.rccl_comm != nullptr, LOOP_EAGER_EXCHANGE},
+        {h->replay.failures >= 3, LOOP_EAGER_GAVE_UP},
+    };
+    for (const auto& r : table) if (r.eager) return r.row;
+    if (h->host_only) return LOOP_REPLAYS;
+    hipStreamCaptureStatus cs = hipStreamCaptureStatusNone;
+    if (s != nullptr && (hipStreamIsCapturing(s, &cs) != hipSuccess || cs != hipStreamCaptureStatusNone)) return LOOP_EAGER_CAPTURING;
+    return LOOP_REPLAYS;
+}
+
+void replay_touched(tgnh_handle h, LoopTouch what) {
+    static const char* const table[TOUCH_COUNT] = {
+                  "tgnh_bind_buffers: other arrays (every launch holds their addresses)",
+                "tgnh_set_step_size (dt of every launch, the chain's sub-step)",
+              "tgnh_set_drude_steps_per_real_step (ChainArgs::S)",
+                "tgnh_set_max_drude_distance (hardwall / max_dist of every launch; the instantiation where it turns on or off)",
+                "tgnh_set_global_dof_terms (the thermostat block is written anew)",
+         "tgnh_set_thermostat_state (a pending chain is run in place first: the handle owes something else afterwards)",
+                 "an exchange attached or detached (who sums the rows, where the chain runs: run_chain's table)",
+           "tgnh_set_resident_share (the grids of step_kernel / wstep_kernel)",
+                    "tgnh_harness_pack_sites / tgnh_harness_lattice_hint (which force kernel, which site tables)",
+                "another x0 / k_drude / k_tether, or the other loop (ForceArgs; the force launch itself)",
+                    "tgnh_set_time (a step's sweep direction is its number's parity)",
+                  "a failure the device reported (nothing more is computed on this trajectory)",
+              "tgnh_set_replay_steps",
+    };
+    if (h->replay.held) h->replay.dropped_by = table[what];
+    h->replay.drop();
+}
+
+static uint32_t loop_state(tgnh_handle h) {
+    return h->owed.bits() | h->owed.chain_pending_twice << 10 | h->owed.carry_pending << 11 | h->owed.tail_summed << 12 | h->owed.end_folded << 13;
+}
+
+static tgnh_status loop_step(tgnh_handle h, const LoopCall& c, void* stream) {
+    tgnh_status rc = tgnh_step_begin(h, stream); if (rc) return rc;
+    if (c.forces) { rc = tgnh_harness_force(h, c.x0, c.k_drude, c.k_tether, const_cast<void*>(h->bound.force), stream); if (rc) return rc; }
+    return tgnh_step_end(h, stream);
+}
+static tgnh_status loop_eager(tgnh_handle h, const LoopCall& c, int nsteps, void* stream) {
+    for (int i = 0; i < nsteps; i++) { tgnh_status rc = loop_step(h, c, stream); if (rc) return rc; }
+    h->replay.eager_steps += nsteps;
+    return TGNH_OK;
+}
+
+static tgnh_status record_loop(tgnh_handle h, const LoopCall& c, bool* steady) {
+    tgnh_context::Replay& R = h->replay;
+    *steady = false;
+    HIP_OK(R.capture.create());
+    const tgnh_context::Owed owed0 = h->owed;
+    const tgnh_context::Run run0 = h->run;
+    const uint32_t key0 = loop_state(h);
+    bool ok = true, periodic = true;
+    tgnh_status rc = TGNH_OK;
+    for (int i = 0; i < 2 && ok; i++) {
+        R.rec[i].parity = (int)(h->run.step_count & 1);
+        if (hipStreamBeginCapture(R.capture, hipStreamCaptureModeThreadLocal) != hipSuccess) { ok = false; break; }
+        for (int k = 0; k < R.K && !rc; k++) rc = loop_step(h, c, (hipStream_t)R.capture);
+        hipGraph_t g = nullptr;
+        const hipError_t e = hipStreamEndCapture(R.capture, &g);
+        ok = !rc && e == hipSuccess && g != nullptr && R.rec[i].exec.instantiate(g) == hipSuccess;
+        if (g) (void)hipGraphDestroy(g);
+        R.rec[i].owed_after = h->owed; R.rec[i].sweep_after = h->run.sweep_reverse;
+        periodic = periodic && loop_state(h) == key0 && (i == 0 || h->run.ke_parts == R.ke_parts);
+        R.ke_parts = h->run.ke_parts;
+    }
+    h->owed = owed0; h->run = run0;
+    if (!ok) (void)hipGetLastError();
+    if (!ok || !periodic || h->status.failed_code) {
+        const int failures = R.failures + (ok ? 0 : 1);
+        R.drop();
+        R.failures = failures;
+        return TGNH_OK;
+    }
+    R.key = key0; R.forces = c.forces; R.x0 = c.x0; R.k_drude = c.k_drude; R.k_tether = c.k_tether;
+    R.held = true; R.failures = 0; R.recordings++;
+    *steady = true;
+    return TGNH_OK;
+}
+
+tgnh_status run_loop(tgnh_handle h, const LoopCall& c, int nsteps, void* stream) {
+    CHECK_H(h);
+    hipStream_t s = (hipStream_t)stream;
+    tgnh_context::Replay& R = h->replay;
+    int left = std::max(nsteps, 0);
+    if (left > 0 && !h->host_only && h->bound.velm && loop_verdict(h, left, s) == LOOP_REPLAYS) {
+        if (R.held && (R.forces != c.forces || (c.forces && (R.x0 != c.x0 || R.k_drude != c.k_drude || R.k_tether != c.k_tether)))) replay_touched(h, TOUCH_LOOP_ARGS);
+        int attempts = 0;
+        while (left >= R.K) {
+            tgnh_status rc;
+            if (!R.held) {
+                if (attempts == 3 || R.failures >= 3) break;
+                attempts++;
+                rc = entry(h, true); if (rc) return rc;
+                bool steady = false;
+                rc = record_loop(h, c, &steady); if (rc) return rc;
+                if (!steady) { rc = loop_eager(h, c, R.K, stream); if (rc) return rc; left -= R.K; }
+                continue;
+            }
+            const int parity = (int)(h->run.step_count & 1);
+            const int turn = R.rec[0].parity == parity ? 0 : (R.rec[1].parity == parity ? 1 : -1);
+            if (turn < 0 || loop_state(h) != R.key) {
+                rc = loop_eager(h, c, 1, stream); if (rc) return rc;
+                left -= 1;
+                continue;
+            }
+            rc = entry(h, true); if (rc) return rc;
+            HIP_OK(hipGraphLaunch(R.rec[turn].exec, s));
+            for (int k = 0; k < R.K; k++) h->run.time += h->d.step_size;
+            h->run.step_count += R.K;
+            h->owed = R.rec[turn].owed_after; h->run.sweep_reverse = R.rec[turn].sweep_after; h->run.ke_parts = R.ke_parts;
+            if (h->status.h_seen) HIP_OK(hipMemcpyAsync(h->status.h_seen, h->status.d_word, sizeof(uint32_t), hipMemcpyDeviceToHost, s));
+            R.launches++;
+            left -= R.K;
+        }
+    }
+    return loop_eager(h, c, left, stream);
+}
+
+extern "C" tgnh_status tgnh_replay_probe(tgnh_handle h, int nsteps, void* stream, int32_t out[6]) {
+    CHECK_H(h);
+    if (!out) return fail(TGNH_ERR_ARG, "null out");
+    const int why = loop_verdict(h, nsteps, (hipStream_t)stream);
+    if (h->host_only && why == LOOP_REPLAYS) h->replay.held = true;
+    out[0] = why; out[1] = h->replay.K; out[2] = h->replay.held ? 1 : 0;
+    out[3] = (int32_t)h->replay.recordings; out[4] = (int32_t)h->replay.launches; out[5] = (int32_t)h->replay.eager_steps;
+    return TGNH_OK;
+}
+
+extern "C" tgnh_status tgnh_set_replay_steps(tgnh_handle h, int steps_per_graph) {
+    CHECK_H(h);
+    if (steps_per_graph < 1) return fail(TGNH_ERR_ARG, "steps per graph must be >= 1");
+    if (steps_per_graph != h->replay.K) replay_touched(h, TOUCH_GRAPH_STEPS);
+    h->replay.K = steps_per_graph;
+    return TGNH_OK;
+}
diff --git a/openmm_drudenose_amd/drudetgnhplugin.py b/openmm_drudenose_amd/drudetgnhplugin.py
--- a/openmm_drudenose_amd/drudetgnhplugin.py
+++ b/openmm_drudenose_amd/drudetgnhplugin.py
@@ -4,7 +4,8 @@
 
 from . import _lib
 from ._lib import (MODE_DUALNH, MODE_TGNH, PREC_SINGLE, PREC_MIXED, PREC_DOUBLE,
-                   FLAG_DEFER_SCALE, FLAG_RESIDENT_STEP, FLAG_WAVE_TILES, FLAG_TRUST_STATE_CHANGED, FLAG_GATHER)
+                   FLAG_DEFER_SCALE, FLAG_RESIDENT_STEP, FLAG_WAVE_TILES, FLAG_TRUST_STATE_CHANGED, FLAG_GATHER,
+                   FLAG_EAGER_LOOPS)
 from .synth import KB
 
 _PREC = {"single": PREC_SINGLE, "mixed": PREC_MIXED, "double": PREC_DOUBLE}
@@ -620,6 +621,17 @@
         replay.graphs = graphs
         return replay
 
+    REPLAY_REASONS = ("replays", "TGNH_FLAG_EAGER_LOOPS", "fewer than 2 K steps", "timing on", "gather path", "exchange attached",
+                      "stream capturing", "recordings failed")
+
+    def replay_probe(self, steps):
+        out = (C.c_int32 * 6)()
+        _check(self.lib.tgnh_replay_probe(self.h, int(steps), self._stream(), out))
+        return dict(reason=self.REPLAY_REASONS[out[0]], K=out[1], held=bool(out[2]), recordings=out[3], graph_launches=out[4], eager_steps=out[5])
+
+    def set_replay_steps(self, k):
+        _check(self.lib.tgnh_set_replay_steps(self.h, int(k)))
+
     def pending_state(self):
         bits = C.c_uint32()
         _check(self.lib.tgnh_get_pending_state(self.h, C.byref(bits)))
```

After: 4011 steps/s. 0.984x the previous value.
